# bcgsc/abyss

Hardware: AMD Instinct MI355X
Metric: Mk-mers/s inserted+extended (abyss-bloom-dbg, k=64); unitig bit-exact (higher is better)
Workload: dtype u64

## Files before the change

abyss_amd/_lib.py:

```python
from __future__ import annotations

import ctypes as C
import os

from . import build

ABG_OK = 0
ABG_EINVAL, ABG_ENODEV, ABG_ENOMEM, ABG_EINTERNAL, ABG_EAGAIN = -1, -2, -3, -4, -5


class Params(C.Structure):
    _fields_ = [
        ("k", C.c_uint32), ("num_hashes", C.c_uint32), ("min_cov", C.c_uint32), ("trim", C.c_uint32),
        ("bloom_bytes", C.c_uint64), ("counters", C.c_uint64), ("spaced_seed", C.c_char_p),
        ("device", C.c_int32), ("verbose", C.c_int32), ("insert_batch_kmers", C.c_uint64),
        ("claim_log2", C.c_uint32), ("walk_slots", C.c_uint32), ("wtab_log2", C.c_uint32),
        ("cascade_levels", C.c_uint32), ("slice_filter", C.c_uint32), ("reserved_", C.c_uint32 * 5),
    ]


class Counters(C.Structure):
    _fields_ = [(n, C.c_uint64) for n in
                ("solid_reads", "visited_reads", "reads_processed", "bases_assembled", "next_contig_id")]


class Contig(C.Structure):
    _fields_ = [
        ("contig_id", C.c_uint64), ("read_index", C.c_uint64), ("seq", C.c_char_p),
        ("length", C.c_uint32), ("coverage", C.c_uint32), ("redundant", C.c_int32),
        ("left_ext", C.c_uint32), ("right_ext", C.c_uint32), ("left_code", C.c_int32),
        ("right_code", C.c_int32), ("seed_pos", C.c_uint32),
    ]


class Stats(C.Structure):
    _fields_ = [(n, C.c_uint64) for n in
                ("insert_rounds", "walk_rounds", "candidates", "walked", "rewalked", "commit_breaks",
                 "commit_rounds", "generated", "bulk_calls", "bulk_steps", "lin_steps", "guide_slots", "chain_steps", "batch_cuts", "overflows", "memo_hits", "memo_adds", "tiled_ops", "tiled_pending", "tile_overflows", "cls_covered_reads", "archive_bases", "cls_decided_reads", "counter_bytes_held",
                 "commit_rounds_incremental", "commit_dirty_records", "commit_first_chunk_decided")]


CONTIG_CB = C.CFUNCTYPE(None, C.c_void_p, C.POINTER(Contig))
TEXT_CB = C.CFUNCTYPE(None, C.c_void_p, C.POINTER(C.c_char), C.c_uint64)

_lib = None


def symbols():
    return [
        "abg_params_init", "abg_create", "abg_destroy", "abg_last_error", "abg_reset", "abg_filter_size",
        "abg_load_seqs", "abg_load_seqs_v", "abg_keep_reads", "abg_assemble_kept", "abg_load_packed", "abg_counting_stats", "abg_counters_export",
        "abg_counters_import", "abg_visited_export", "abg_visited_import", "abg_assemble_seqs", "abg_assemble_seqs_v",
        "abg_assemble_packed", "abg_cascade_export", "abg_get_counters", "abg_set_counters", "abg_hash_seq",
        "abg_contains_seq",
        "abg_attach_comm", "abg_share_reads", "abg_rccl_unique_id", "abg_rccl_comm_create", "abg_rccl_comm_destroy",
        "abg_dev_copy", "abg_dev_alloc", "abg_dev_free", "abg_output_graph_seqs",
        "abg_profile_enable", "abg_profile_reset", "abg_profile_get", "abg_get_stats",
        "abg_overlap_create", "abg_overlap_destroy", "abg_overlap_last_error", "abg_overlap_join", "abg_overlap_edges",
        "abg_overlap_profile", "abg_overlap_profile_get",
        "abg_rr_create", "abg_rr_destroy", "abg_rr_last_error", "abg_rr_bytes", "abg_rr_clear", "abg_rr_insert_seqs",
        "abg_rr_contains_seqs", "abg_rr_popcount", "abg_rr_export", "abg_rr_sync", "abg_rr_profile", "abg_rr_profile_get",
        "abg_kn_create", "abg_kn_destroy", "abg_kn_last_error", "abg_kn_import", "abg_kn_export", "abg_kn_insert_seqs",
        "abg_kn_contains_seqs", "abg_kn_popcount", "abg_kn_hash_seq", "abg_kn_sync", "abg_kn_profile", "abg_kn_profile_get",
        "abg_fm_create", "abg_fm_destroy", "abg_fm_last_error", "abg_fm_build", "abg_fm_size", "abg_fm_export", "abg_fm_map_seqs",
        "abg_fm_sync", "abg_fm_tune", "abg_fm_profile", "abg_fm_profile_get",
        "abg_de_create", "abg_de_destroy", "abg_de_last_error", "abg_de_set_pmf", "abg_de_scan", "abg_de_estimate", "abg_de_tune",
        "abg_de_profile", "abg_de_profile_get",
        "abg_ov_create", "abg_ov_destroy", "abg_ov_last_error", "abg_ov_set_contigs", "abg_ov_find", "abg_ov_profile",
        "abg_ov_profile_get",
        "abg_sg_create", "abg_sg_destroy", "abg_sg_last_error", "abg_sg_set_graph", "abg_sg_search", "abg_sg_tune", "abg_sg_profile",
        "abg_sg_profile_get",
        "abg_mc_create", "abg_mc_destroy", "abg_mc_last_error", "abg_mc_set_contigs", "abg_mc_merge", "abg_mc_tune", "abg_mc_profile",
        "abg_mc_profile_get",
        "abg_pb_create", "abg_pb_destroy", "abg_pb_last_error", "abg_pb_tune", "abg_pb_align", "abg_pb_align_chain", "abg_pb_profile_get",
        "abg_pb_profile_reset",
    ]


def load(path: str | None = None):
    global _lib
    if _lib is not None:
        return _lib
    if path is None:
        path = os.environ.get("ABG_LIB") or build.LIB
        if not os.path.exists(path):
            build.build_lib()
    lib = C.CDLL(path)
    vp, u64p, u8p = C.c_void_p, C.POINTER(C.c_uint64), C.c_void_p
    lib.abg_params_init.argtypes = [C.POINTER(Params)]
    lib.abg_params_init.restype = None
    lib.abg_create.argtypes = [C.POINTER(Params), C.POINTER(vp)]
    lib.abg_destroy.argtypes = [vp]
    lib.abg_destroy.restype = None
    lib.abg_last_error.argtypes = [vp]
    lib.abg_last_error.restype = C.c_char_p
    lib.abg_reset.argtypes = [vp]
    lib.abg_contains_seq.argtypes = [vp, C.c_char_p, C.c_uint64, vp, vp, C.c_uint64, u64p]
    lib.abg_filter_size.argtypes = [vp, u64p]
    lib.abg_load_seqs.argtypes = [vp, C.c_char_p, vp, C.c_uint64]
    lib.abg_load_packed.argtypes = [vp, vp, vp, vp, C.c_uint64]
    lib.abg_load_seqs_v.argtypes = [vp, C.c_uint32, vp, vp, vp]
    lib.abg_keep_reads.argtypes = [vp, C.c_int, C.c_uint64]
    lib.abg_assemble_kept.argtypes = [vp, vp, CONTIG_CB, vp]
    lib.abg_counting_stats.argtypes = [vp, u64p, u64p]
    lib.abg_counters_export.argtypes = [vp, u8p]
    lib.abg_counters_import.argtypes = [vp, u8p]
    lib.abg_visited_export.argtypes = [vp, u8p]
    lib.abg_visited_import.argtypes = [vp, u8p]
    lib.abg_assemble_seqs.argtypes = [vp, C.c_char_p, vp, C.c_uint64, vp, CONTIG_CB, vp]
    lib.abg_assemble_seqs_v.argtypes = [vp, C.c_uint32, vp, vp, vp, vp, CONTIG_CB, vp]
    lib.abg_assemble_packed.argtypes = [vp, vp, vp, vp, C.c_uint64, vp, CONTIG_CB, vp]
    lib.abg_cascade_export.argtypes = [vp, C.c_uint32, u8p]
    lib.abg_get_counters.argtypes = [vp, C.POINTER(Counters)]
    lib.abg_set_counters.argtypes = [vp, C.POINTER(Counters)]
    lib.abg_hash_seq.argtypes = [vp, C.c_char_p, C.c_uint64, vp, vp, C.c_uint64, u64p]
    lib.abg_profile_enable.argtypes = [vp, C.c_int]
    lib.abg_profile_reset.argtypes = [vp]
    lib.abg_profile_get.argtypes = [vp, C.c_char_p, C.POINTER(C.c_double), u64p]
    lib.abg_get_stats.argtypes = [vp, C.POINTER(Stats)]
    lib.abg_attach_comm.argtypes = [vp, vp]
    lib.abg_share_reads.argtypes = [vp, vp, vp, vp, C.c_uint64, C.POINTER(vp), C.POINTER(vp), C.POINTER(vp), u64p]
    lib.abg_rccl_unique_id.argtypes = [vp]
# ... 109 lines not shown
```

abyss_amd/build.py:

```python
from __future__ import annotations

import os
import shutil
import subprocess
import sys

ROOT = os.path.dirname(os.path.dirname(os.path.abspath(__file__)))
CSRC = os.path.join(ROOT, "abyss_amd", "csrc")
LIB = os.path.join(ROOT, "abyss_amd", "lib", "libabyss_amd.so")
BIN_DIR = os.path.join(ROOT, "abyss_amd", "bin")
ORACLE_DIR = os.path.join(ROOT, "oracle")
HOSTCHECK = os.path.join(ROOT, "tests", "hostcheck", "libhostcheck.so")
REFERENCE = "/root/reference"


def _newer(target: str, sources) -> bool:
    if not os.path.exists(target):
        return True
    t = os.path.getmtime(target)
    return any(os.path.getmtime(s) > t for s in sources if os.path.exists(s))


def _run(cmd, cwd=None):
    r = subprocess.run(cmd, cwd=cwd, stdout=subprocess.PIPE, stderr=subprocess.STDOUT, text=True)
# ... 23 lines not shown
    "abg_fm": ["abg_fm.hip", "abg_fm.h", "abg_core.h"],
    "abg_de": ["abg_de.hip", "abg_de.h", "abg_core.h"],
    "abg_ov": ["abg_ov.hip", "abg_ov.h", "abg_core.h"],
    "abg_sg": ["abg_sg.hip", "abg_sg.h", "abg_core.h"],
    "abg_mc": ["abg_mc.hip", "abg_mc.h", "abg_ov.h", "abg_core.h"],
    "abg_pb": ["abg_pb.hip", "abg_pb.h", "abg_mc.h", "abg_ov.h", "abg_core.h"],
}
UNIT_FLAGS = {"abg_de": ["-ffp-contract=off"]}


def build_lib(force: bool = False) -> str:
    os.makedirs(OBJ_DIR, exist_ok=True)
    header = os.path.join(ROOT, "include", "abyss_amd.h")
    objs, procs = [], []
    for unit, deps in UNITS.items():
        obj = os.path.join(OBJ_DIR, unit + ".o")
        objs.append(obj)
        if force or _newer(obj, [os.path.join(CSRC, d) for d in deps] + [header]):
            cmd = [hipcc(), "--offload-arch=gfx950", "-O3", "-std=c++17", "-fPIC"] + UNIT_FLAGS.get(unit, []) + \
                ["-c", "-o", obj, os.path.join(CSRC, unit + ".hip")]
            procs.append((cmd, subprocess.Popen(cmd, stdout=subprocess.PIPE, stderr=subprocess.STDOUT, text=True)))
    for cmd, p in procs:
        out, _ = p.communicate()
        if p.returncode != 0:
            sys.stderr.write(out)
            raise RuntimeError("build step failed: %s" % " ".join(cmd))
    if force or procs or _newer(LIB, objs):
        _run([hipcc(), "--offload-arch=gfx950", "-shared", "-fPIC", "-o", LIB] + objs)
    return LIB


def build_cli(force: bool = False) -> str:
    src = os.path.join(CSRC, "host", "bloom_dbg_main.cc")
    out = os.path.join(BIN_DIR, "abyss-bloom-dbg")
    if not os.path.exists(src):
        return ""
    deps = [src] + [os.path.join(CSRC, "host", f) for f in os.listdir(os.path.join(CSRC, "host"))]
    if force or _newer(out, deps + [LIB]):
        os.makedirs(BIN_DIR, exist_ok=True)
        build_lib()
        _run(["g++", "-std=c++17", "-O2", "-I" + os.path.join(ROOT, "include"), "-o", out, src,
              "-L" + os.path.dirname(LIB), "-labyss_amd", "-Wl,-rpath,$ORIGIN/../lib", "-lpthread"])
        _run(["g++", "-std=c++17", "-O2", "-I" + os.path.join(ROOT, "include"), "-o",
              os.path.join(BIN_DIR, "abyss-bloom"), os.path.join(CSRC, "host", "bloom_main.cc"),
              "-L" + os.path.dirname(LIB), "-labyss_amd", "-Wl,-rpath,$ORIGIN/../lib", "-lpthread"])
        _run(["g++", "-std=c++17", "-O2", "-I" + os.path.join(ROOT, "include"), "-o",
              os.path.join(BIN_DIR, "AdjList"), os.path.join(CSRC, "host", "adjlist_main.cc"),
              "-L" + os.path.dirname(LIB), "-labyss_amd", "-Wl,-rpath,$ORIGIN/../lib", "-lpthread"])
        _run(["g++", "-std=c++17", "-O2", "-I" + os.path.join(ROOT, "include"), "-o",
              os.path.join(BIN_DIR, "abyss-rresolver-short"), os.path.join(CSRC, "host", "rresolver_main.cc"),
              "-L" + os.path.dirname(LIB), "-labyss_amd", "-Wl,-rpath,$ORIGIN/../lib", "-lpthread"])
        for name, main in (("abyss-map", "map_main.cc"), ("abyss-index", "index_main.cc"), ("DistanceEst", "distanceest_main.cc"),
                           ("Overlap", "overlap_main.cc"), ("SimpleGraph", "simplegraph_main.cc"), ("MergeContigs", "mergecontigs_main.cc"),
                           ("PopBubbles", "popbubbles_main.cc")):
            _run(["g++", "-std=c++17", "-O2", "-I" + os.path.join(ROOT, "include"), "-o",
                  os.path.join(BIN_DIR, name), os.path.join(CSRC, "host", main),
                  "-L" + os.path.dirname(LIB), "-labyss_amd", "-Wl,-rpath,$ORIGIN/../lib", "-lpthread"] +
                 (["-ffp-contract=off"] if name == "DistanceEst" else []))
    return out


def build_oracle(force: bool = False) -> None:
    targets = ["oracle"]
    if os.path.isdir(REFERENCE):
        targets.append("ref")
    if force:
        _run(["make", "-C", ORACLE_DIR, "clean"])
    _run(["make", "-C", ORACLE_DIR, "-j8"] + targets)


READER_CHECK = os.path.join(ROOT, "tests", "hostcheck", "reader_check")
ADJLIST_CHECK = os.path.join(ROOT, "tests", "hostcheck", "adjlist_check")
RRESOLVER_CHECK = os.path.join(ROOT, "tests", "hostcheck", "rresolver_check")
KN_CHECK = os.path.join(ROOT, "tests", "hostcheck", "kn_check")
FM_CHECK = os.path.join(ROOT, "tests", "hostcheck", "fm_check")
DE_CHECK = os.path.join(ROOT, "tests", "hostcheck", "de_check")
OV_CHECK = os.path.join(ROOT, "tests", "hostcheck", "ov_check")
SG_CHECK = os.path.join(ROOT, "tests", "hostcheck", "sg_check")
MC_CHECK = os.path.join(ROOT, "tests", "hostcheck", "mc_check")
PB_CHECK = os.path.join(ROOT, "tests", "hostcheck", "pb_check")


def build_hostcheck(force: bool = False) -> str:
    src = os.path.join(ROOT, "tests", "hostcheck", "hostcheck_ext.cc")
    if force or _newer(HOSTCHECK, [src, os.path.join(ROOT, "tests", "hostcheck", "hostcheck.cc")] + csrc_files()):
        _run(["g++", "-std=c++17", "-O2", "-g", "-fPIC", "-shared", "-Wno-unknown-pragmas", "-o", HOSTCHECK, src])
    rsrc = os.path.join(ROOT, "tests", "hostcheck", "reader_check.cc")
    if force or _newer(READER_CHECK, [rsrc, os.path.join(CSRC, "host", "fasta_reader.h")]):
        _run(["g++", "-std=c++17", "-O2", "-o", READER_CHECK, rsrc])
    asrc = os.path.join(ROOT, "tests", "hostcheck", "adjlist_check.cc")
    if force or _newer(ADJLIST_CHECK, [asrc, HOSTCHECK, os.path.join(CSRC, "host", "adjlist_core.h"),
                                       os.path.join(CSRC, "host", "fasta_reader.h")]):
        _run(["g++", "-std=c++17", "-O2", "-o", ADJLIST_CHECK, asrc, "-L" + os.path.dirname(HOSTCHECK), "-lhostcheck",
              "-Wl,-rpath,$ORIGIN"])
    hsrc = [os.path.join(CSRC, "host", f) for f in ("rresolver_core.h", "graph_writers.h", "fasta_reader.h", "si_bytes.h")]
    csrc = os.path.join(ROOT, "tests", "hostcheck", "rresolver_check.cc")
    if force or _newer(RRESOLVER_CHECK, [csrc, os.path.join(CSRC, "abg_rr.h"), os.path.join(CSRC, "abg_core.h")] + hsrc):
        _run(["g++", "-std=c++17", "-O2", "-Wno-unknown-pragmas", "-o", RRESOLVER_CHECK, csrc, "-lpthread"])
    ksrc = os.path.join(ROOT, "tests", "hostcheck", "kn_check.cc")
    kdeps = [ksrc] + [os.path.join(CSRC, f) for f in ("abg_kn.h", "abg_core.h")] + \
        [os.path.join(CSRC, "host", f) for f in ("bloom_core.h", "fasta_reader.h")]
    if force or _newer(KN_CHECK, kdeps):
        _run(["g++", "-std=c++17", "-O2", "-Wno-unknown-pragmas", "-o", KN_CHECK, ksrc, "-lpthread"])
    fsrc = os.path.join(ROOT, "tests", "hostcheck", "fm_check.cc")
    fdeps = [fsrc] + [os.path.join(CSRC, f) for f in ("abg_fm.h", "abg_core.h")] + \
        [os.path.join(CSRC, "host", f) for f in ("map_core.h", "fasta_reader.h")]
    if force or _newer(FM_CHECK, fdeps):
        _run(["g++", "-std=c++17", "-O2", "-Wno-unknown-pragmas", "-o", FM_CHECK, fsrc, "-lpthread"])
    dsrc = os.path.join(ROOT, "tests", "hostcheck", "de_check.cc")
    ddeps = [dsrc] + [os.path.join(CSRC, f) for f in ("abg_de.h", "abg_core.h")] + [os.path.join(CSRC, "host", "distanceest_core.h")]
    if force or _newer(DE_CHECK, ddeps):
        _run(["g++", "-std=c++17", "-O2", "-ffp-contract=off", "-Wno-unknown-pragmas", "-o", DE_CHECK, dsrc, "-lpthread"])
    osrc = os.path.join(ROOT, "tests", "hostcheck", "ov_check.cc")
    odeps = [osrc] + [os.path.join(CSRC, f) for f in ("abg_ov.h", "abg_core.h")] + \
        [os.path.join(CSRC, "host", f) for f in ("overlap_core.h", "rresolver_core.h", "graph_writers.h", "fasta_reader.h", "si_bytes.h")]
    if force or _newer(OV_CHECK, odeps):
        _run(["g++", "-std=c++17", "-O2", "-Wno-unknown-pragmas", "-o", OV_CHECK, osrc, "-lpthread"])
    ssrc = os.path.join(ROOT, "tests", "hostcheck", "sg_check.cc")
    sdeps = [ssrc] + [os.path.join(CSRC, f) for f in ("abg_sg.h", "abg_core.h")] + \
        [os.path.join(CSRC, "host", f) for f in ("simplegraph_core.h", "overlap_core.h", "rresolver_core.h", "graph_writers.h", "fasta_reader.h", "si_bytes.h")]
    if force or _newer(SG_CHECK, sdeps):
        _run(["g++", "-std=c++17", "-O2", "-Wno-unknown-pragmas", "-o", SG_CHECK, ssrc, "-lpthread"])
    msrc = os.path.join(ROOT, "tests", "hostcheck", "mc_check.cc")
    mdeps = [msrc] + [os.path.join(CSRC, f) for f in ("abg_mc.h", "abg_ov.h", "abg_core.h")] + \
        [os.path.join(CSRC, "host", f) for f in ("mergecontigs_core.h", "overlap_core.h", "rresolver_core.h", "graph_writers.h", "fasta_reader.h", "si_bytes.h")]
    if force or _newer(MC_CHECK, mdeps):
        _run(["g++", "-std=c++17", "-O2", "-Wno-unknown-pragmas", "-o", MC_CHECK, msrc, "-lpthread"])
    psrc = os.path.join(ROOT, "tests", "hostcheck", "pb_check.cc")
    pdeps = [psrc] + [os.path.join(CSRC, f) for f in ("abg_pb.h", "abg_mc.h", "abg_ov.h", "abg_core.h")] + \
        [os.path.join(CSRC, "host", f) for f in ("popbubbles_core.h", "rresolver_core.h", "graph_writers.h", "fasta_reader.h", "si_bytes.h")]
    if force or _newer(PB_CHECK, pdeps):
        _run(["g++", "-std=c++17", "-O2", "-Wno-unknown-pragmas", "-o", PB_CHECK, psrc, "-lpthread"])
    return HOSTCHECK


def build_all(force: bool = False) -> None:
    build_lib(force)
    build_cli(force)
    build_oracle(force)
    build_hostcheck(force)


if __name__ == "__main__":
    build_all("--force" in sys.argv)
    print("built:", LIB)
```

abyss_amd/csrc/abg_core.h:

```cpp
#pragma once

#include <stdint.h>
#include <stddef.h>

#if defined(__HIPCC__)
#include <hip/hip_runtime.h>
#define ABG_HD __host__ __device__ __forceinline__
#define ABG_HDN __host__ __device__
#define ABG_HDX __host__ __device__ __attribute__((noinline))
#else
#define ABG_HD inline
#define ABG_HDN
#define ABG_HDX
#endif

namespace abg {

constexpr int MAX_NW = 6;
constexpr int MAX_HASHES = 32;
constexpr unsigned FP_TRIM = 5;

enum Dir : int { FORWARD = 0, REVERSE = 1 };
enum Sense : int { SENSE = 0, ANTISENSE = 1 };

// ... 1035 lines not shown
}

#if defined(__HIP_DEVICE_COMPILE__)
ABG_HD uint64_t ld_coherent(const uint64_t* p)
{
	return __hip_atomic_load(p, __ATOMIC_RELAXED, __HIP_MEMORY_SCOPE_AGENT);
}
ABG_HD uint32_t ld_coherent(const uint32_t* p)
{
	return __hip_atomic_load(p, __ATOMIC_RELAXED, __HIP_MEMORY_SCOPE_AGENT);
}
ABG_HD void st_coherent(uint64_t* p, uint64_t v)
{
	__hip_atomic_store(p, v, __ATOMIC_RELAXED, __HIP_MEMORY_SCOPE_AGENT);
}
ABG_HD uint64_t cas_u64(uint64_t* p, uint64_t expect, uint64_t val)
{
	return (uint64_t)atomicCAS((unsigned long long*)p, (unsigned long long)expect,
	    (unsigned long long)val);
}
ABG_HD uint32_t cas_u32(uint32_t* p, uint32_t expect, uint32_t val) { return atomicCAS(p, expect, val); }
ABG_HD uint32_t atomic_min_u32(uint32_t* p, uint32_t v) { return atomicMin(p, v); }
ABG_HD uint64_t atomic_min_u64(uint64_t* p, uint64_t v)
{
	return (uint64_t)atomicMin((unsigned long long*)p, (unsigned long long)v);
}
ABG_HD uint32_t atomic_add_u32(uint32_t* p, uint32_t v) { return atomicAdd(p, v); }
ABG_HD uint64_t atomic_add_u64(uint64_t* p, uint64_t v)
{
	return (uint64_t)atomicAdd((unsigned long long*)p, (unsigned long long)v);
}
ABG_HD uint32_t atomic_or_u32(uint32_t* p, uint32_t v) { return atomicOr(p, v); }
ABG_HD uint64_t atomic_exch_u64(uint64_t* p, uint64_t v)
{
	return (uint64_t)atomicExch((unsigned long long*)p, (unsigned long long)v);
}
#else
ABG_HD uint64_t ld_coherent(const uint64_t* p) { return *p; }
ABG_HD uint32_t ld_coherent(const uint32_t* p) { return *p; }
ABG_HD void st_coherent(uint64_t* p, uint64_t v) { *p = v; }
ABG_HD uint64_t cas_u64(uint64_t* p, uint64_t expect, uint64_t val)
{
	uint64_t old = *p;
	if (old == expect) *p = val;
	return old;
}
ABG_HD uint32_t cas_u32(uint32_t* p, uint32_t expect, uint32_t val) { uint32_t o = *p; if (o == expect) *p = val; return o; }
ABG_HD uint32_t atomic_min_u32(uint32_t* p, uint32_t v) { uint32_t o = *p; if (v < o) *p = v; return o; }
ABG_HD uint64_t atomic_min_u64(uint64_t* p, uint64_t v) { uint64_t o = *p; if (v < o) *p = v; return o; }
ABG_HD uint32_t atomic_add_u32(uint32_t* p, uint32_t v) { uint32_t o = *p; *p = o + v; return o; }
ABG_HD uint64_t atomic_add_u64(uint64_t* p, uint64_t v) { uint64_t o = *p; *p = o + v; return o; }
ABG_HD uint32_t atomic_or_u32(uint32_t* p, uint32_t v) { uint32_t o = *p; *p = o | v; return o; }
ABG_HD uint64_t atomic_exch_u64(uint64_t* p, uint64_t v) { uint64_t o = *p; *p = v; return o; }
#endif

#if defined(__HIP_DEVICE_COMPILE__)
ABG_HD uint32_t wave_append_slot(uint32_t* counter, bool want)
{
	const uint64_t m = __ballot(want ? 1 : 0);
	if (m == 0) return 0;
	const unsigned lane = __lane_id();
	const int leader = __ffsll((unsigned long long)m) - 1;
	uint32_t base = 0;
	if ((int)lane == leader) base = atomicAdd(counter, (uint32_t)__popcll(m));
	base = (uint32_t)__shfl((int)base, leader);
	return base + (uint32_t)__popcll(m & ((1ull << lane) - 1));
}
#else
ABG_HD uint32_t wave_append_slot(uint32_t* counter, bool want)
{
	if (!want) return 0;
	uint32_t o = *counter; *counter = o + 1; return o;
}
#endif

#if defined(__HIP_DEVICE_COMPILE__)
ABG_HD void wave_count_add(uint64_t* counter, bool want)
{
	const uint64_t m = __ballot(want ? 1 : 0);
	if (m && (int)__lane_id() == __ffsll((unsigned long long)m) - 1) atomicAdd((unsigned long long*)counter, (unsigned long long)__popcll(m));
}
#else
ABG_HD void wave_count_add(uint64_t* counter, bool want) { if (want) *counter += 1; }
#endif

#if defined(__HIP_DEVICE_COMPILE__)
ABG_HD uint32_t wave_rank(bool want, uint32_t& count)
{
	const uint64_t m = __ballot(want ? 1 : 0);
	count = (uint32_t)__popcll(m);
	return (uint32_t)__popcll(m & ((1ull << __lane_id()) - 1));
}
#else
ABG_HD uint32_t wave_rank(bool want, uint32_t& count) { count = want ? 1u : 0u; return 0; }
#endif

#if defined(__HIP_DEVICE_COMPILE__)
ABG_HD void wave_put_bit(uint64_t* words, uint32_t i, bool v)
{
	const uint64_t m = __ballot(v ? 1 : 0);
	if (!(i & 63u)) words[i >> 6] = m;
}
#else
ABG_HD void wave_put_bit(uint64_t* words, uint32_t i, bool v)
{
	if (!(i & 63u)) words[i >> 6] = 0;
	words[i >> 6] |= (uint64_t)(v ? 1u : 0u) << (i & 63u);
}
#endif

#if defined(__HIP_DEVICE_COMPILE__)
ABG_HD uint64_t wu_cas_u64(uint64_t* p, uint64_t expect, uint64_t val, bool coop)
{
	if (!coop) return cas_u64(p, expect, val);
	uint64_t r = 0;
	if (__lane_id() == 0) r = cas_u64(p, expect, val);
	return ((uint64_t)(uint32_t)__builtin_amdgcn_readfirstlane((int)(r >> 32)) << 32) |
	       (uint32_t)__builtin_amdgcn_readfirstlane((int)(uint32_t)r);
}
ABG_HD uint32_t wu_atomic_min_u32(uint32_t* p, uint32_t v, bool coop)
{
	if (!coop) return atomic_min_u32(p, v);
	uint32_t r = 0;
	if (__lane_id() == 0) r = atomic_min_u32(p, v);
	return (uint32_t)__builtin_amdgcn_readfirstlane((int)r);
}
ABG_HD uint32_t wu_atomic_add_u32(uint32_t* p, uint32_t v, bool coop)
{
	if (!coop) return atomic_add_u32(p, v);
	uint32_t r = 0;
	if (__lane_id() == 0) r = atomic_add_u32(p, v);
	return (uint32_t)__builtin_amdgcn_readfirstlane((int)r);
}
ABG_HD uint64_t wu_atomic_add_u64(uint64_t* p, uint64_t v, bool coop)
{
	if (!coop) return atomic_add_u64(p, v);
	uint64_t r = 0;
	if (__lane_id() == 0) r = atomic_add_u64(p, v);
	return ((uint64_t)(uint32_t)__builtin_amdgcn_readfirstlane((int)(r >> 32)) << 32) |
	       (uint32_t)__builtin_amdgcn_readfirstlane((int)(uint32_t)r);
}
ABG_HD void wu_st_coherent(uint64_t* p, uint64_t v, bool coop)
{
	if (!coop || __lane_id() == 0) st_coherent(p, v);
}
ABG_HD void wu_st_u32(uint32_t* p, uint32_t v, bool coop)
{
	if (!coop || __lane_id() == 0) *p = v;
}
ABG_HD void wu_st_u8(uint8_t* p, uint8_t v, bool coop)
{
	if (!coop || __lane_id() == 0) *p = v;
}
#else
ABG_HD void wu_st_coherent(uint64_t* p, uint64_t v, bool) { st_coherent(p, v); }
ABG_HD void wu_st_u32(uint32_t* p, uint32_t v, bool) { *p = v; }
ABG_HD void wu_st_u8(uint8_t* p, uint8_t v, bool) { *p = v; }
ABG_HD uint64_t wu_cas_u64(uint64_t* p, uint64_t e, uint64_t v, bool) { return cas_u64(p, e, v); }
ABG_HD uint32_t wu_atomic_min_u32(uint32_t* p, uint32_t v, bool) { return atomic_min_u32(p, v); }
ABG_HD uint32_t wu_atomic_add_u32(uint32_t* p, uint32_t v, bool) { return atomic_add_u32(p, v); }
ABG_HD uint64_t wu_atomic_add_u64(uint64_t* p, uint64_t v, bool) { return atomic_add_u64(p, v); }
#endif

struct Guide {
	const uint64_t* tab;
	uint64_t mask;
// ... 966 lines not shown
```

abyss_amd/csrc/abg_engine.h:

```cpp
#pragma once
#include "abg_walk.h"

#include <algorithm>
#include <chrono>
#include <cstdio>
#include <cstdlib>
#include <cstring>
#include <functional>
#include <future>
#include <string>
#include <type_traits>
#include <vector>

namespace abg {

struct Failure { int code; std::string msg; };
constexpr int FAIL_INVAL = -1, FAIL_NOMEM = -3, FAIL_INTERNAL = -4;
[[noreturn]] inline void fail_now(int code, const std::string& msg) { throw Failure{ code, msg }; }
inline std::string strf(const char* fmt, unsigned long long a = 0, unsigned long long b = 0)
{
	char buf[256];
	snprintf(buf, sizeof buf, fmt, a, b);
	return buf;
}

struct Config {
	uint32_t k = 0, nh = 4, kc = 2, trim = 0;
	uint64_t counters = 0;
	uint32_t cascade_levels = 0;
	std::string spaced_seed;
	uint64_t insert_batch_kmers = 1ull << 24;
	uint32_t claim_log2 = 30;
	uint32_t drain_threshold = 1u << 12;
	uint64_t compact_threshold = 1u << 20;
	bool async_load = true;
	bool tiled_insert = true;
	bool benign_sharers = true;
	uint32_t cls_debug_skip = 0;
	bool cls_archive = true;
	uint32_t cls_archive_max_mb = 16384;
	bool sorted_overflow = true;
	bool cosettle = true;
	uint32_t cosettle_passes = 6;
	uint32_t cosettle_log2 = 24;
	uint32_t walk_slots = 4096;
	uint32_t tb_cap = 512;
	uint32_t buf_cap = 1u << 16;
	uint64_t pool_cap = 1ull << 28;
	uint32_t rec_cap = 1u << 22;
	uint32_t wtab_log2 = 26;
	uint32_t wtab_log2_max = 31;
	uint32_t cend_log2 = 20;
	uint64_t p2_first_batch = 65536;
	uint64_t p2_max_batch = 1ull << 22;
	uint32_t p2_growth = 2;
	uint32_t p2_crowded = 1u << 18;
	uint32_t p2_starved_growth = 2;
	uint32_t p2_starved = 6144;
	uint32_t slice_filter = 0;
	bool solid_plane = true;
	uint32_t classify_slots = 65536;
	uint32_t cls_both_max_mb = 1024;
	bool cls_both = true;
	bool prefetch_classify = true;
	uint32_t memo_log2 = 0;
	bool memo = true;
	uint32_t p2_max_candidates = 1u << 18;
	uint32_t t_tags = 1024;
	uint32_t commit_incremental = 1;
	uint32_t commit_dirty_max = 4096;
	uint32_t commit_dirty_log2 = 26;
	uint32_t guide_stride = 4;
	uint32_t guide_log2_max = 31;
	bool guide_seen = true;
	bool link_duplicates = true;
	bool par_commit = true;
	bool overlap_bins = true;
	bool overlap_purity = true;
	bool apply_mask = true;
	bool lead_implicit = true;
	uint32_t dist_hash_all_ranks = 2;
	uint32_t dist_route_min_ranks = 4;
	uint64_t keep_insert_scratch_bytes = 16ull << 30;
	uint64_t par_commit_max_bytes = 16ull << 30;
	int verbose = 0;
};

struct Counters {
	uint64_t solid_reads = 0, visited_reads = 0, reads_processed = 0, bases_assembled = 0,
	         contig_id = 0;
};

struct BaseCodes {
	uint8_t t[256];
	BaseCodes()
	{
		for (int i = 0; i < 256; i++) t[i] = 0xFF;
		t['A'] = t['a'] = 0; t['C'] = t['c'] = 1; t['G'] = t['g'] = 2; t['T'] = t['t'] = 3;
	}
};
template <class T>
struct NoInitAlloc : std::allocator<T> {
	template <class U> struct rebind { using other = NoInitAlloc<U>; };
	template <class U, class... A> void construct(U* p, A&&... a)
	{
		if constexpr (sizeof...(A) == 0) ::new ((void*)p) U; else ::new ((void*)p) U(std::forward<A>(a)...);
	}
};
struct HostBatch {
	std::vector<uint32_t, NoInitAlloc<uint32_t>> words;
	std::vector<uint64_t> woff{ 0 };
	std::vector<uint32_t> len;
	std::vector<uint64_t> koff{ 0 };
	void clear() { words.clear(); woff.assign(1, 0); len.clear(); koff.assign(1, 0); }
	uint64_t n() const { return len.size(); }
	void add_ascii(const char* s, uint32_t L, uint32_t k)
	{
		static const BaseCodes codes;
		uint64_t w0 = words.size();
		words.resize(w0 + (L + 15) / 16);
		uint32_t* out = words.data() + w0;
		uint32_t i = 0;
		for (; i + 16 <= L; i += 16) {
			uint32_t w = 0;
			for (uint32_t j = 0; j < 16; j++) w |= (uint32_t)(codes.t[(unsigned char)s[i + j]] & 3u) << (2 * j);
			*out++ = w;
		}
		if (i < L) {
			uint32_t w = 0;
			for (uint32_t j = 0; i + j < L; j++) w |= (uint32_t)(codes.t[(unsigned char)s[i + j]] & 3u) << (2 * j);
			*out = w;
		}
		woff.push_back(words.size());
		len.push_back(L);
		koff.push_back(koff.back() + (L - k + 1));
	}
};

struct ContigOut {
	uint64_t contig_id;
	uint64_t read_index;
	std::string seq;
	uint32_t coverage;
	bool redundant;
	uint32_t left_ext, right_ext;
	int left_code, right_code;
	uint32_t seed_pos;
};

ABG_HD uint64_t claim_val(uint32_t epoch, uint32_t t) { return ((uint64_t)(0xFFFFFFFFu - epoch) << 32) | t; }

struct FHash {
	Params p; Batch b; uint64_t* h0;
	ABG_HD void operator()(uint64_t t, uint32_t) const
	{
		uint64_t r = find_seq(b.koff, b.n, t);
		uint32_t j = (uint32_t)(t - b.koff[r]);
		h0[t] = scratch_hash(p, [&](unsigned i) { return batch_base(b, r, j + i); });
// ... 1533 lines not shown
	{
		const uint32_t L = b.len[r];
		if (L < p.k) return;
		const uint32_t nk = L - p.k + 1;
		const uint64_t woff = b.woff[r];
		if (nk > GUIDE_MAX_NK || woff > GUIDE_MAX_WOFF) return;
		if (!p.mask) {
			constexpr uint32_t RUN = 8;
			for (uint32_t j0 = lane * RUN; j0 < nk; j0 += nlanes * RUN) {
				const uint32_t j1 = j0 + RUN < nk ? j0 + RUN : nk;
				uint64_t hm[RUN];
				for (uint32_t q = 0; q < RUN; q++) hm[q] = 0;
				kmer_hash_run(p, [&](unsigned q) { return batch_base(b, r, q); }, j0, j1, [&](uint32_t j, uint64_t h) { hm[j - j0] = h; });
				unsigned c[RUN];
#pragma unroll
				for (uint32_t q = 0; q < RUN; q++) c[q] = probe_c(p, cnt, pos_i(p, hm[j0 + q < j1 ? q : 0u], 0));
#pragma unroll
				for (uint32_t q = 0; q < RUN; q++)
					if (j0 + q < j1 && c[q] >= p.kc) tab[guide_slot(hm[q], mask)] = guide_pack(woff, j0 + q, nk, guide_tag(hm[q]));
			}
			return;
		}
		for (uint32_t j = lane; j < nk; j += nlanes) {
			const Kmer<NW> s = window_kmer<NW>(b.words, woff, j, p.k);
			uint64_t fh, rh;
			kmer_hashes(s, p.k, fh, rh);
			const uint64_t hm = rh < fh ? rh : fh;
			uint64_t df = 0, dr = 0;
			if constexpr (MASKED_BUILD<NW>) masked_terms(p, s, df, dr);
			const uint64_t fs = fh ^ df, rs = rh ^ dr;
			if (probe_c(p, cnt, pos_i(p, rs < fs ? rs : fs, 0)) < p.kc) continue;
			tab[guide_slot(hm, mask)] = guide_pack(woff, j, nk, guide_tag(hm));
		}
	}
};

constexpr uint32_t WALK_FAST_WITH_CACHE = 16384;
template <int NW>
struct FWalk {
	WalkEnv<NW> e; const uint32_t* list;
	ABG_HDN void operator()(uint64_t i, uint32_t slot, void* fast, uint32_t fast_bytes, bool coop)
	{
		WalkEnv<NW>* env = (WalkEnv<NW>*)fast;
		const uint32_t a = (uint32_t)((sizeof(WalkEnv<NW>) + 15) & ~15ull);
		*env = e;
		env->mcache = nullptr;
		if (fast_bytes >= WALK_FAST_WITH_CACHE) {
			fast_bytes -= (uint32_t)sizeof(MaskCache);
			env->mcache = (MaskCache*)((char*)fast + fast_bytes);
		}
		env->fast = (char*)fast + a;
		env->fast_bytes = fast_bytes - a;
		env->coop = coop;
		walk_read<NW>(*env, list[i], slot);
	}
};

template <int NW>
ABG_HDN uint64_t seq_kmer_hash(const Params& p, const uint8_t* seq, uint64_t j)
{
	return scratch_hash(p, [&](unsigned i) { return (unsigned)seq[j + i]; });
}
template <int NW>
ABG_HDN uint64_t read_kmer_hash(const Params& p, const Batch& b, uint64_t r, uint32_t j)
{
	return scratch_hash(p, [&](unsigned i) { return batch_base(b, r, j + i); });
}
constexpr uint32_t PREP_RUN = 8;
ABG_HD uint64_t dup_mix(uint64_t x) { x ^= x >> 31; x *= 0xD6E8FEB86659FD93ULL; x ^= x >> 29; x *= 0x9E3779B97F4A7C15ULL; x ^= x >> 32; return x | 1; }
template <int NW>
struct FReadPrep {
	Params p; Batch b; const uint32_t* cand_read; const uint64_t* rkoff; uint64_t* rkh; uint32_t first;
	ABG_HDN void operator()(uint64_t i, uint32_t lane, uint32_t nlanes) const
	{
		uint32_t c = first + (uint32_t)i;
		uint64_t r = cand_read[c];
		uint32_t nk = b.len[r] - p.k + 1;
		uint64_t* out = rkh + rkoff[c];
		for (uint32_t j0 = lane * PREP_RUN; j0 < nk; j0 += nlanes * PREP_RUN)
			kmer_hash_run(p, [&](unsigned q) { return batch_base(b, r, q); }, j0, j0 + PREP_RUN < nk ? j0 + PREP_RUN : nk,
			    [&](uint32_t j, uint64_t h) { out[j] = h; });
	}
};
template <int NW>
struct FContigPrep {
	Params p; const uint8_t* cnt; ContigRec* recs; uint32_t first; const uint8_t* pool; uint64_t* kh;
	uint32_t with_cov;
	ABG_HDN void operator()(uint64_t i, uint32_t lane, uint32_t nlanes) const
	{
		ContigRec& rec = recs[first + i];
		const uint8_t* seq = pool + rec.seq_off;
		uint64_t* out = kh + rec.seq_off;
		uint32_t cnk = rec.len - p.k + 1;
		uint32_t cov = 0;
		uint64_t fp = 0;
		for (uint32_t j0 = lane * PREP_RUN; j0 < cnk; j0 += nlanes * PREP_RUN)
			kmer_hash_run(p, [&](unsigned q) { return (unsigned)seq[q]; }, j0, j0 + PREP_RUN < cnk ? j0 + PREP_RUN : cnk,
			    [&](uint32_t j, uint64_t h) { out[j] = h; fp += dup_mix(h); if (with_cov) cov += solid_min_count(p, cnt, h); });
		if (cov) atomic_add_u32(&rec.coverage, cov);
		if (fp) atomic_add_u64(&rec.fp, fp);
	}
};

struct FDupKeys {
	const ContigRec* recs; uint32_t k; uint64_t* key; uint32_t* val;
	ABG_HD void operator()(uint64_t i, uint32_t) const
	{
		const ContigRec& r = recs[i];
		key[i] = r.len < k + FP_TRIM - 1 ? ~0ULL - i : dup_mix(r.fp ^ ((uint64_t)r.len << 40));
		val[i] = (uint32_t)i;
	}
};
struct FDupLink {
	ContigRec* recs; const uint64_t* key; const uint32_t* val; uint64_t n; uint32_t first_new;
	ABG_HD void operator()(uint64_t q, uint32_t) const
	{
		const uint32_t me = val[q];
		if (me < first_new) return;
		const uint64_t k = key[q];
		uint64_t g = q;
		for (unsigned s = 0; s < 64 && g > 0 && key[g - 1] == k; s++) g--;
		uint32_t best = REC_END, best_cand = recs[me].cand;
		for (unsigned s = 0; s < 128 && g < n && key[g] == k; s++, g++) {
			const uint32_t o = val[g];
			if (o != me && recs[o].cand < best_cand && recs[o].len == recs[me].len && recs[o].fp == recs[me].fp) { best = o; best_cand = recs[o].cand; }
		}
		recs[me].dup_of = best;
	}
};
struct FDupVerify {
	ContigRec* recs; const uint64_t* kh; uint32_t k; uint32_t first_new;
	ABG_HDN void operator()(uint64_t i, uint32_t lane, uint32_t nlanes) const
	{
		ContigRec& d = recs[first_new + i];
		const uint32_t o = d.dup_of;
		if (o == REC_END) return;
		const uint64_t* a = kh + d.seq_off; const uint64_t* b = kh + recs[o].seq_off;
		const uint32_t nk = d.len - k + 1;
		bool fwd = true, rev = true;
		for (uint32_t j = lane; j < nk; j += nlanes) { const uint64_t x = a[j]; fwd = fwd & (x == b[j]); rev = rev & (x == b[nk - 1 - j]); }
		fwd = wave_all_lanes(fwd, nlanes); rev = wave_all_lanes(rev, nlanes);
		if (!fwd && !rev && lane == 0) d.dup_of = REC_END;
	}
};
constexpr uint32_t PC_SCAN_RUN = 4;
template <class Test>
ABG_HD bool wave_all_kmers(uint32_t n, uint32_t lane, uint32_t nlanes, Test test, bool& first_chunk)
{
	bool mine = lane < n ? test(lane) : true;
	first_chunk = !wave_all_lanes(mine, nlanes);
	if (first_chunk) return false;
	for (uint32_t j0 = nlanes; j0 < n; j0 += PC_SCAN_RUN * nlanes) {
#pragma unroll
		for (uint32_t u = 0; u < PC_SCAN_RUN; u++) {
			const uint32_t j = j0 + u * nlanes + lane;
			if (j < n) mine = mine & test(j);
		}
		if (!wave_all_lanes(mine, nlanes)) return false;
	}
	return true;
}
ABG_HD bool visited_contains_owned(const Params& p, const uint8_t* __restrict__ vis, uint64_t h, uint64_t lo, uint64_t span)
{
	bool ok = true;
	if (p.nh <= 4) {
		uint64_t q4[4]; uint8_t b4[4];
#pragma unroll
		for (unsigned i = 0; i < 4; i++) { q4[i] = pos_i(p, h, i < p.nh ? i : 0u); b4[i] = vis[q4[i] >> 3]; }
#pragma unroll
		for (unsigned i = 0; i < 4; i++) if (i < p.nh && q4[i] - lo < span) ok = ok & (((b4[i] >> (q4[i] & 7)) & 1u) != 0);
		return ok;
	}
	for (unsigned i = 0; i < p.nh; i++) {
		const uint64_t q = pos_i(p, h, i);
		if (q - lo < span) ok = ok & (((vis[q >> 3] >> (q & 7)) & 1u) != 0);
	}
	return ok;
}
template <int NW>
struct FPreCommit {
	Params p; Batch b; const uint32_t* cand_read; const uint32_t* status; const uint32_t* first_rec;
	ContigRec* recs; const uint8_t* vis; const uint64_t* kh; const uint64_t* rkh; const uint64_t* rkoff;
	uint8_t* read_flag; uint32_t first;
	uint64_t lo, span; uint8_t* part_c; uint8_t* part_r;
	uint32_t* nfirst;
	ABG_HDN void operator()(uint64_t i, uint32_t lane, uint32_t nlanes) const
	{
		uint32_t c = first + (uint32_t)i;
		uint64_t r = cand_read[c];
		uint32_t nk = b.len[r] - p.k + 1;
		const uint64_t* rh = rkh + rkoff[c];
		bool fc;
		const bool all = wave_all_kmers(nk, lane, nlanes, [&](uint32_t j) { return visited_contains_owned(p, vis, rh[j], lo, span); }, fc);
		uint32_t nf = fc ? 1u : 0u;
		if (nfirst && lane == 0) nfirst[i] = nf;
		if (part_c) {
			if (lane == 0) part_c[i] = all ? 1 : 0;
			if (status[c] != WS_COMPLETE) return;
		} else {
			if (lane == 0) read_flag[c] = all ? 1 : 0;
			if (all || status[c] != WS_COMPLETE) return;
		}
		for (uint32_t ri = first_rec[c]; ri != REC_END; ri = recs[ri].next) {
			ContigRec& rec = recs[ri];
			uint32_t cnk = rec.len - p.k + 1;
			if (rec.len < p.k + FP_TRIM - 1 || rec.pre_redundant) continue;
			if (rec.dup_of != REC_END && recs[rec.dup_of].cand >= first) continue;
			const uint64_t* ch = kh + rec.seq_off;
			const bool red = wave_all_kmers(cnk, lane, nlanes, [&](uint32_t j) { return visited_contains_owned(p, vis, ch[j], lo, span); }, fc);
			nf += fc ? 1u : 0u;
			if (part_r) { if (lane == 0) part_r[ri] = red ? 1 : 0; }
			else if (lane == 0 && red) rec.pre_redundant = 1;
		}
		if (nfirst && lane == 0) nfirst[i] = nf;
	}
};
struct FPreCommitCopies {
	const uint32_t* status; const uint32_t* first_rec; ContigRec* recs; const uint8_t* read_flag; uint32_t first; uint32_t k;
	ABG_HD void operator()(uint64_t i, uint32_t) const
	{
		const uint32_t c = first + (uint32_t)i;
		if (read_flag[c] || status[c] != WS_COMPLETE) return;
		for (uint32_t ri = first_rec[c]; ri != REC_END; ri = recs[ri].next) {
			ContigRec& rec = recs[ri];
			if (rec.len < k + FP_TRIM - 1 || rec.pre_redundant || rec.dup_of == REC_END) continue;
// ... 847 lines not shown
				kmin[rec.seq_off + j] = (uint8_t)mn;
			}
			if (sum && cov) atomic_add_u32(&rec.coverage, cov);
		}
	}
};
struct FPcWrite {
	ParCommit e; uint32_t* order; uint32_t order_base; uint64_t id_base;
	ABG_HD void operator()(uint64_t i, uint32_t) const
	{
		const uint32_t c = e.c_begin + (uint32_t)i;
		if (c >= e.brk || !e.active[i]) return;
		uint32_t o = order_base + e.cnt[i];
		uint64_t id = id_base + e.cnt2[i];
		for (uint32_t ri = e.first_rec[c]; ri != REC_END; ri = e.recs[ri].next) {
			ContigRec& rec = e.recs[ri];
			order[o++] = ri;
			if (rec.ins) rec.contig_id = id++;
		}
	}
};

template <class BE>
class Engine {
  public:
	Engine(BE& be, const Config& cfg) : be_(be), cfg_(cfg)
	{
		uint64_t rem = cfg_.counters % 8;
		m_ = rem ? cfg_.counters + 8 - rem : cfg_.counters;
		p_ = make_params(cfg_.k, cfg_.nh, cfg_.kc, cfg_.trim, m_);
		if (!cfg_.spaced_seed.empty()) {
			MaskTab* mt = new MaskTab;
			make_mask(cfg_.spaced_seed.c_str(), cfg_.k, *mt, p_);
			mask_d_ = (MaskTab*)be_.alloc(sizeof(MaskTab));
			be_.h2d(mask_d_, mt, sizeof(MaskTab));
			delete mt;
			p_.mask = mask_d_;
		}
		if (cfg_.cascade_levels) {
			casc_.levels = cfg_.cascade_levels;
			casc_.level_words = (m_ + 31) / 32;
			casc_.bits = (uint32_t*)be_.alloc(casc_.levels * casc_.level_words * 4);
			be_.memset(casc_.bits, 0, casc_.levels * casc_.level_words * 4);
			cnt_ = (uint8_t*)be_.alloc(8);
			vis_bytes_ = 8;
		} else {
			const uint64_t dev = be_.device_mem_bytes();
			cnt_deferred_ = cfg_.slice_filter == 1 || (cfg_.slice_filter == 0 && dev && (double)m_ * 1.3 > (double)dev * 0.9);
			if (!cnt_deferred_) {
				cnt_ = (uint8_t*)be_.alloc(m_ + 64 * (MAX_RANKS + 1));
				be_.memset(cnt_, 0, m_);
			}
			vis_bytes_ = (m_ / 8 + 4 + 3) & ~3ull;
		}
		vis_ = (uint8_t*)be_.alloc(vis_bytes_);
		be_.memset(vis_, 0, vis_bytes_);
		cstate_ = (CommitState*)be_.alloc(sizeof(CommitState));
		be_.memset(cstate_, 0, sizeof(CommitState));
		scal_ = (uint64_t*)be_.alloc(64);
	}
	~Engine()
	{
		if (BE::ITEM_GROUP_LOG2 == 0 && getenv("ABG_LEAD_COUNT"))
			fprintf(stderr, "lead_stores made=%llu skipped=%llu\n", (unsigned long long)stats_.lead_stores[0], (unsigned long long)stats_.lead_stores[1]);
		free_counters(); be_.free(vis_); if (both_) be_.free(both_); be_.free(cstate_); be_.free(scal_);
		free_archive();
		if (casc_.bits) be_.free(casc_.bits);
		if (mask_d_) be_.free(mask_d_);
		if (T_) be_.free(T_);
		if (Tk_) { be_.free(Tk_); be_.free(Tv_); }
		if (pcA_) be_.free(pcA_);
		if (la_pool_c_) be_.free(la_pool_c_);
		if (la_pool_c2_) be_.free(la_pool_c2_);
		if (guide_tab_) be_.free(guide_tab_);
		if (guide_seen_) be_.free(guide_seen_);
		if (gtab_.hmin) free_tab(gtab_);
		free_shared();
		free_insert();
		free_walk();
		if (cend_.hmin) free_tab(cend_);
		if (memo_tab_.hmin) free_tab(memo_tab_);
		if (plane_) be_.free(plane_);
		if (wstats_) be_.free(wstats_);
	}
	void reset()
	{
		if (casc_.bits) be_.memset(casc_.bits, 0, casc_.levels * casc_.level_words * 4);
		else if (sliced_) be_.memset(cnt_ + own_lo_, 0, own_span_);
		else if (cnt_) be_.memset(cnt_, 0, m_);
		be_.memset(vis_, 0, vis_bytes_);
		arc_valid_ = false; loaded_ops_ = 0;
		be_.memset(cstate_, 0, sizeof(CommitState));
		counters_ = Counters();
		stats_ = Stats();
		cnt_partial_ = false; cnt_loaded_ = false;
		memo_valid_ = false; plane_valid_ = false;
		last_rounds_ = 0;
		p2_batch_ = cfg_.p2_first_batch;
		last_candidates_ = 0;
		if (cend_.hmin) {
			be_.memset(cend_.hmin, 0xFF, (cend_.mask + 1) * 8);
			be_.memset(cend_.meta, 0xFF, (cend_.mask + 1) * 8);
		}
		cend_count_ = 0;
		if (wstats_) clear_wstats();
		ovf_seen_[0] = ovf_seen_[1] = 0;
		if (gtab_.hmin) { free_tab(gtab_); gtab_ = WalkTab{ nullptr, nullptr, nullptr, 0 }; gtab_used_ = 0; }
	}
	const Params& params() const { return p_; }
	uint64_t size() const { return m_; }
	uint8_t* counters_dev() { need_whole_filter("direct access to the counters"); gather_counters(); memo_valid_ = false; plane_valid_ = false; arc_valid_ = false;  return cnt_; }

	struct Comm {
		int rank = 0, world = 1;
		bool stream_ordered = false;
		void* user = nullptr;
		int (*all_gather_v)(void*, void*, const uint64_t*, const uint64_t*, void*) = nullptr;
		int (*all_reduce)(void*, void*, uint64_t, int32_t, int32_t, void*) = nullptr;
		int (*all_to_all_v)(void*, const void*, const uint64_t*, const uint64_t*, void*, const uint64_t*, const uint64_t*, void*) = nullptr;
	};
	enum { DT_U8 = 0, DT_U32 = 1, DT_U64 = 2, OP_SUM = 0, OP_MAX = 1, OP_MIN = 2 };
	bool attach_comm(const Comm& c)
	{
		if (c.world < 1 || c.world > MAX_RANKS || c.rank < 0 || c.rank >= c.world || casc_.bits) return false;
		uint64_t chunk = (m_ + c.world - 1) / c.world;
		chunk = (chunk + 63) & ~63ull;
		if (sliced_ && cnt_loaded_ && (c.rank != comm_.rank || c.world != comm_.world))
			fail_now(FAIL_INVAL, "a sliced filter that holds counters cannot take a communicator with another rank or world (abg_counters_export / _import move them)");
		const bool keep_window = sliced_ && c.rank == comm_.rank && c.world == comm_.world && own_chunk_ == chunk;
		comm_ = c;
		free_insert();
		own_lo_ = std::min<uint64_t>(m_, (uint64_t)c.rank * chunk);
		own_span_ = std::min<uint64_t>(m_, own_lo_ + chunk) - own_lo_;
		own_chunk_ = chunk;
		if (sliced_ || cnt_deferred_) {
			if (!cfg_.solid_plane || (m_ & 63) || !cfg_.par_commit)
				fail_now(FAIL_INVAL, "a sliced filter needs the bit plane, the parallel commit and a multiple of 64 counters");
			if (!keep_window) {
				free_counters();
				if (plane_) { be_.free(plane_); plane_ = nullptr; }
				win_total_ = (uint64_t)c.world * chunk + 64;
				win_span_ = chunk + 64;
				win_lo_ = own_lo_;
				cnt_ = (uint8_t*)be_.alloc_window(win_total_, win_lo_, win_span_);
				be_.memset(cnt_ + own_lo_, 0, win_span_);
				cnt_loaded_ = false;
			}
			sliced_ = true; cnt_deferred_ = false;
			cfg_.drain_threshold = 0;
			memo_valid_ = false; plane_valid_ = false;
		}
		const char* f = getenv("ABG_FORCE_DIST");
		force_dist_ = f && atoi(f) != 0;
		if (c.world > 1 && !comm_scaled_) {
			comm_scaled_ = true;
			cfg_.p2_first_batch *= (uint64_t)c.world;
			cfg_.p2_max_batch *= (uint64_t)c.world;
			cfg_.p2_starved *= (uint32_t)c.world;
			cfg_.p2_crowded *= (uint32_t)std::min(c.world, 4);
			p2_batch_ = cfg_.p2_first_batch;
		}
		return true;
	}
	bool dist() const { return comm_.world > 1 || force_dist_ || sliced_; }
	bool sliced() const { return sliced_; }
	uint64_t counter_bytes_held() const { return sliced_ ? win_span_ : cnt_ ? m_ : 0; }
	void need_counters() const
	{
		if (!cnt_) fail_now(FAIL_INVAL, "this filter does not fit the device: attach a communicator first, its ranks keep a range each (abg_attach_comm)");
	}
	void need_whole_filter(const char* what) const
	{
		need_counters();
		if (sliced_) fail_now(FAIL_INVAL, std::string(what) + " is not available on a sliced filter (each rank holds a range of the counters)");
	}
	void free_counters()
	{
		if (sliced_) be_.free_window(cnt_, win_total_, win_lo_, win_span_);
		else if (cnt_) be_.free(cnt_);
		cnt_ = nullptr; sliced_ = false;
	}
	Batch share_reads(const Batch& loc)
	{
		const uint32_t R = (uint32_t)comm_.world, me = (uint32_t)comm_.rank;
		uint64_t w0 = 0, w1 = 0;
		if (loc.n) { be_.d2h(&w0, loc.woff, 8); be_.d2h(&w1, loc.woff + loc.n, 8); }
		std::vector<uint64_t> cnt(2 * R, 0);
		cnt[2 * me] = loc.n; cnt[2 * me + 1] = w1 - w0;
// ... 322 lines not shown
	{
		const bool want = cfg_.cls_archive && !dist() && !sliced_ && !casc_.bits && b.n && use_par_commit();
		if (!want) { free_archive(); return; }
		const uint64_t nk = loaded_ops_ ? loaded_ops_ : m_ / 4;
		uint64_t cap = std::max<uint64_t>(nk / 4, 1ull << 16) + ARC_HEAD, slots = 1ull << 12;
		while (slots < cap / 2) slots <<= 1;
		const uint64_t budget = (uint64_t)cfg_.cls_archive_max_mb << 20;
		while (slots > (1ull << 12) && slots * 8 + cap > budget) { slots >>= 1; cap = std::min(cap, slots * 2); }
		if (cap >= (1ULL << ARC_POS_BITS)) cap = (1ULL << ARC_POS_BITS) - 1;
		if (arc_.seq && (arc_.cap < cap || arc_.mask + 1 < slots)) free_archive();
		if (!arc_.seq) {
			arc_.seq = (uint8_t*)be_.try_alloc(cap + ARC_PAD);
			arc_.tab = (uint64_t*)be_.try_alloc(slots * 8);
			arc_.used = (uint64_t*)be_.try_alloc(8);
			if (!arc_.seq || !arc_.tab || !arc_.used) {
				if (arc_.seq) be_.free(arc_.seq); if (arc_.tab) be_.free(arc_.tab); if (arc_.used) be_.free(arc_.used);
				arc_ = ContigArchive();
				return;
			}
			arc_.cap = cap; arc_.mask = slots - 1;
			arc_valid_ = false;
		}
		arc_.nreads = wstats_ ? wstats_ + WSTAT_CLS_COVERED : nullptr;
		if (!arc_valid_) {
			be_.memset(arc_.seq, ARC_SEP, arc_.cap + ARC_PAD);
			be_.memset(arc_.tab, 0, (arc_.mask + 1) * 8);
			const uint64_t head = ARC_HEAD;
			be_.h2d(arc_.used, &head, 8);
			arc_valid_ = true;
		}
	}
	ContigArchive arc_{}; bool arc_valid_ = false;
	uint64_t loaded_ops_ = 0;
	uint64_t ovf_seen_[2] = { 0, 0 };
	uint8_t* plane_ = nullptr; bool plane_valid_ = false;
	Params p2_; const uint8_t* cnt2_ = nullptr;

	void build_guide(const Batch& b)
	{
		guide_.tab = nullptr; guide_.seen = nullptr; guide_slots_ = 0;
		if (!cfg_.guide_stride || p_.nh > 8 || !b.n) return;
		const uint64_t sampled = (b.n + cfg_.guide_stride - 1) / cfg_.guide_stride;
		uint64_t nwords = 0;
		be_.d2h(&nwords, b.woff + b.n, 8);
		const uint64_t bases = nwords * 16, minus = b.n * (uint64_t)(p_.k - 1);
		const uint64_t kmers = (bases > minus ? bases - minus : b.n) / std::min<uint32_t>(cfg_.guide_stride, 4u);
		uint32_t log2 = 16;
		while ((1ull << log2) < kmers && log2 < cfg_.guide_log2_max) log2++;
		if (!guide_tab_ || log2 != guide_log2_) {
			if (guide_tab_) be_.free(guide_tab_);
			guide_tab_ = (uint64_t*)be_.try_alloc(8ull << log2);
			guide_log2_ = log2;
			if (!guide_tab_) { if (cfg_.verbose) fprintf(stderr, "abyss_amd: no memory for the walkers' guide table, walking step by step\n"); return; }
		}
		be_.memset(guide_tab_, 0, 8ull << log2);
		guide_.mask = (1ull << log2) - 1; guide_.words = b.words; guide_.nwords = nwords;
		dispatch_nw([&](auto nw) {
			FGuideBuild<decltype(nw)::value> f{ p2_, b, cnt2_, guide_tab_, guide_.mask, cfg_.guide_stride, sampled };
			be_.launch_wave((sampled + GUIDE_READS_PER_ITEM - 1) / GUIDE_READS_PER_ITEM, f, "guide_build");
		});
		guide_.tab = guide_tab_;
		guide_slots_ = guide_.mask + 1;
		if (cfg_.guide_seen) {
			const uint64_t need = nwords * 16, total = be_.device_mem_bytes();
			if (guide_seen_ && guide_seen_bytes_ < need) { be_.free(guide_seen_); guide_seen_ = nullptr; }
			if (!guide_seen_ && (!total || need <= total / 24)) { guide_seen_ = (uint8_t*)be_.try_alloc(need); guide_seen_bytes_ = need; }
			if (guide_seen_) { be_.memset(guide_seen_, 0, need); guide_.seen = guide_seen_; }
		}
	}
	uint64_t next_batch_size() const
	{
		if (last_candidates_ > cfg_.p2_crowded) return std::max<uint64_t>(p2_batch_ / 2, 1024);
		if (last_candidates_ < cfg_.p2_starved) return std::min<uint64_t>(p2_batch_ * cfg_.p2_starved_growth, 8 * cfg_.p2_max_batch);
		return std::min<uint64_t>(p2_batch_ * cfg_.p2_growth, cfg_.p2_max_batch);
	}
	void clear_wstats()
	{
		be_.memset(wstats_, 0, WSTAT_N * 8);
	}
	struct Stats { uint64_t rounds = 0, walked = 0, rewalked = 0, candidates = 0, breaks = 0, insert_rounds = 0, commit_rounds = 0, generated = 0;
	               uint64_t bulk_calls = 0, bulk_steps = 0, lin_steps = 0, guide_slots = 0, chain_steps = 0, batch_cuts = 0, overflows = 0, memo_hits = 0, memo_adds = 0;
	               uint64_t tiled_ops = 0, tiled_pending = 0, tile_overflows = 0, cls_covered_reads = 0, archive_bases = 0, cls_decided_reads = 0;
	               uint64_t lead_stores[2] = { 0, 0 };
	               uint64_t commit_rounds_incremental = 0, commit_dirty_records = 0, commit_first_chunk_decided = 0; };
	Stats stats()
	{
		Stats s = stats_;
		if (wstats_) {
			uint64_t v[WSTAT_N];
			be_.d2h(v, wstats_, sizeof v);
			s.bulk_calls = v[WSTAT_BULK_CALLS]; s.bulk_steps = v[WSTAT_BULK_STEPS]; s.lin_steps = v[WSTAT_LIN_STEPS]; s.chain_steps = v[WSTAT_CHAIN_STEPS];
			s.memo_hits = v[WSTAT_MEMO_HITS]; s.memo_adds = v[WSTAT_MEMO_ADDS];
			s.cls_covered_reads = v[WSTAT_CLS_COVERED]; s.cls_decided_reads = v[WSTAT_CLS_DECIDED];
		}
		if (arc_.seq && arc_valid_) { uint64_t u = 0; be_.d2h(&u, arc_.used, 8); s.archive_bases = std::min(u, arc_.cap) - ARC_HEAD; }
		s.guide_slots = guide_slots_;
		return s;
	}

  private:
	BE& be_;
	Config cfg_;
	Params p_;
	uint64_t m_ = 0, vis_bytes_ = 0;
	uint8_t* cnt_ = nullptr;
	uint8_t* vis_ = nullptr;
	CommitState* cstate_ = nullptr;
	uint64_t* scal_ = nullptr;
	Cascade casc_{ nullptr, 0, 0 };
	MaskTab* mask_d_ = nullptr;
	std::chrono::steady_clock::time_point dbg_t0_;
	uint32_t* T_ = nullptr;
	uint32_t t_tag_ = 0;
	uint64_t* Tk_ = nullptr; uint32_t* Tv_ = nullptr; uint32_t Tlog2_ = 0;
	uint64_t T_entries_ = 0;
	uint32_t* pcA_ = nullptr; uint64_t pcA_bits_ = 0; uint32_t pcA_shift_ = 0;
	bool t_hashed() const { return t_force_hashed_ || m_ * 4ull > cfg_.par_commit_max_bytes; }
	bool t_force_hashed_ = false;
	bool use_par_commit()
	{
		if (!cfg_.par_commit || t_failed_) return false;
		if (t_hashed()) return true;
		if (!T_) {
			T_ = (uint32_t*)be_.try_alloc(m_ * 4ull);
			t_tag_ = 0;
			if (!T_ && sliced_) {
				t_force_hashed_ = true;
				if (cfg_.verbose) fprintf(stderr, "abyss_amd: no memory for a time stamp per filter bit, hashed stamps instead\n");
				return true;
			}
			if (!T_) { t_failed_ = true; if (cfg_.verbose) fprintf(stderr, "abyss_amd: no memory for the parallel commit's time stamps, using the ordered kernel\n"); return false; }
		}
		return true;
	}
	bool t_failed_ = false;
	Comm comm_;
	bool force_dist_ = false, comm_scaled_ = false;
	bool sliced_ = false, cnt_deferred_ = false; uint64_t win_total_ = 0, win_span_ = 0, win_lo_ = 0;
	bool cnt_loaded_ = false;
	uint64_t own_lo_ = 0, own_span_ = 0, own_chunk_ = 0;
	uint8_t* tred_ = nullptr;
	bool cnt_partial_ = false;
	uint32_t* sh_words_ = nullptr; uint64_t* sh_woff_ = nullptr; uint32_t* sh_len_ = nullptr; uint64_t* sh_koff_ = nullptr;
	uint8_t* dres_ = nullptr; uint8_t* dlost_ = nullptr;
	TilePair* rsend_ = nullptr; TilePair* rrecv_ = nullptr; uint32_t rcap_ = 0; uint64_t rrecv_cap_ = 0; uint32_t* rslot_ = nullptr; uint32_t* rcur_ = nullptr;
	uint8_t* rrep_out_ = nullptr; uint8_t* rrep_in_ = nullptr; uint8_t* rtgt_out_ = nullptr; uint8_t* rtgt_in_ = nullptr; uint8_t* rpendf_ = nullptr;
	uint64_t rown_ = 0;
	bool routed() const
	{
		return dist() && cfg_.dist_route_min_ranks && (uint32_t)comm_.world >= cfg_.dist_route_min_ranks && (comm_.all_to_all_v || comm_.world == 1) && p_.nh <= 16;
	}
	uint32_t g_rec_ = 0; uint64_t g_pool_ = 0;
  public:
  private:
	void free_shared()
	{
		if (!sh_words_) return;
		be_.free(sh_words_); be_.free(sh_woff_); be_.free(sh_len_); be_.free(sh_koff_);
		sh_words_ = nullptr;
	}
	void c_fail(const char* what) { fail_now(FAIL_INTERNAL, std::string("collective ") + what + " failed on rank " + std::to_string(comm_.rank)); }
	void c_all_gather_v(void* buf, const uint64_t* counts, const uint64_t* displs)
	{
		if (!comm_.stream_ordered) be_.sync();
		be_.begin("comm_all_gather");
		if (comm_.all_gather_v(comm_.user, buf, counts, displs, be_.stream_handle())) c_fail("all_gather_v");
		be_.end("comm_all_gather");
	}
	void c_all_reduce(void* buf, uint64_t n, int dtype, int op)
	{
		if (!n) return;
		if (!comm_.stream_ordered) be_.sync();
		be_.begin("comm_all_reduce");
		if (comm_.all_reduce(comm_.user, buf, n, dtype, op, be_.stream_handle())) c_fail("all_reduce");
		be_.end("comm_all_reduce");
	}
	void c_all_to_all_v(const void* send, const uint64_t* sc, const uint64_t* sd, void* recv, const uint64_t* rc, const uint64_t* rd)
	{
		if (comm_.world == 1) {
			if (sc[0]) be_.d2d((char*)recv + rd[0], (const char*)send + sd[0], sc[0]);
			return;
		}
		if (!comm_.stream_ordered) be_.sync();
		be_.begin("comm_all_to_all");
		if (comm_.all_to_all_v(comm_.user, send, sc, sd, recv, rc, rd, be_.stream_handle())) c_fail("all_to_all_v");
		be_.end("comm_all_to_all");
	}
	void host_all_reduce_sum(uint64_t* v, uint32_t n)
	{
		uint64_t* d = (uint64_t*)be_.alloc(n * 8ull);
		be_.h2d(d, v, n * 8ull);
		c_all_reduce(d, n, DT_U64, OP_SUM);
		be_.d2h(v, d, n * 8ull);
		be_.free(d);
	}
	void gather_counters()
	{
		if (!dist() || !cnt_partial_ || sliced_) return;
		std::vector<uint64_t> c(comm_.world), d(comm_.world);
		for (int q = 0; q < comm_.world; q++) { d[q] = (uint64_t)q * own_chunk_; c[q] = own_chunk_; }
		c_all_gather_v(cnt_, c.data(), d.data());
		cnt_partial_ = false;
	}
	Counters counters_;
	Stats stats_;
	uint64_t last_rounds_ = 0;
	uint64_t p2_batch_ = 0;
	uint64_t* h0_ = nullptr; uint64_t* claim_[2] = { nullptr, nullptr };
	uint32_t* pend_[2] = { nullptr, nullptr }; uint32_t* pend_n_ = nullptr; uint32_t epoch_ = 1;
	uint64_t batch_ops_ = 0;
	uint32_t hash_run_ = 8;
	uint64_t insert_scratch_bytes_ = 0;
	uint32_t claim_log2_ = 0;
	bool tiled_ = false; uint64_t ntiles_ = 0, napply_ = 0; uint32_t tile_cap_ = 0;
	TilePair* coarse_ = nullptr; uint32_t* ccur_ = nullptr; uint32_t coarse_cap_ = 0, cshift_ = 0, ncoarse_ = 0;
	TilePair* bins_ = nullptr; uint32_t* tcur_ = nullptr; uint32_t* lead_ = nullptr; uint8_t* opflag_ = nullptr; uint8_t* tgt_ = nullptr; uint8_t* pendf_ = nullptr;
	uint64_t* h0_alt_ = nullptr; TilePair* bins_alt_ = nullptr; uint32_t* tcur_alt_ = nullptr;
	uint32_t* colist_ = nullptr; uint8_t* cocnt_ = nullptr;
	uint64_t* pgrp_ = nullptr;
	uint8_t* wmask_ = nullptr; uint32_t* bad_ = nullptr; uint32_t* cochg_ = nullptr;
	uint32_t* lead_alt_ = nullptr; uint8_t* opflag_alt_ = nullptr;
	uint64_t* amask_ = nullptr; uint64_t* amask_alt_ = nullptr;
	bool staged_purity_ = false;
	Guide guide_{ nullptr, 0, nullptr, 0, nullptr }; uint64_t* guide_tab_ = nullptr; uint32_t guide_log2_ = 0;
	uint8_t* guide_seen_ = nullptr; uint64_t guide_seen_bytes_ = 0;
	BulkScratch* bulk_pool_ = nullptr; uint64_t* wstats_ = nullptr; uint64_t guide_slots_ = 0;
	SuccMemo memo_{ nullptr, nullptr, nullptr, 0 }; WalkTab memo_tab_{ nullptr, nullptr, nullptr, 0 }; bool memo_valid_ = false; uint64_t memo_gen_ = 0;
	bool walk_ready_ = false;
	WalkTab wtab_{}, cend_{ nullptr, nullptr, nullptr, 0 };
	uint32_t wtab_log2_ = 0;
	uint64_t wtab_per_walker_ = 1536;
	void* tb_pool_ = nullptr; VKey* tbk_pool_ = nullptr; VKey* la_pool_ = nullptr; uint8_t* lbuf_ = nullptr; uint8_t* rbuf_ = nullptr;
	uint8_t* pool_ = nullptr; uint64_t pool_cap_ = 0; uint64_t* pool_used_ = nullptr;
	ContigRec* recs_ = nullptr; uint32_t rec_cap_ = 0; uint32_t* rec_used_ = nullptr;
	uint32_t* order_ = nullptr; uint32_t* order_n_ = nullptr;
	uint32_t walk_tb_cap_ = 0, walk_buf_cap_ = 0, wslots_ = 0, cslots_ = 0;
	uint64_t* kh_ = nullptr; uint64_t* rkh_ = nullptr; uint64_t* dbg_ = nullptr;
	uint64_t cend_count_ = 0;
	uint8_t* read_flag_ = nullptr;
	uint64_t last_candidates_ = 0;
	VKey* la_pool_c_ = nullptr;
	VKey* la_pool_c2_ = nullptr;
	uint64_t pre_first_ = 0, pre_n_ = 0;
	std::function<void()> prefetch_;

	WalkTab gtab_{ nullptr, nullptr, nullptr, 0 };
	uint64_t gtab_used_ = 0;
	template <class F>
	void dispatch_nw(F&& f)
	{
		switch (p_.mask ? NW_MASKED + p_.nw : p_.nw) {
		case 1: f(std::integral_constant<int, 1>()); break;
		case 2: f(std::integral_constant<int, 2>()); break;
		case 3: f(std::integral_constant<int, 3>()); break;
		case 4: f(std::integral_constant<int, 4>()); break;
		case 5: case 6: f(std::integral_constant<int, 6>()); break;
		case NW_MASKED + 1: f(std::integral_constant<int, NW_MASKED + 1>()); break;
		case NW_MASKED + 2: f(std::integral_constant<int, NW_MASKED + 2>()); break;
		case NW_MASKED + 3: f(std::integral_constant<int, NW_MASKED + 3>()); break;
		case NW_MASKED + 4: f(std::integral_constant<int, NW_MASKED + 4>()); break;
		default: f(std::integral_constant<int, NW_MASKED + 6>()); break;
		}
	}
	template <int NW>
	void graph_bfs_nw(const Batch& starts, const Batch& marks, std::vector<uint8_t>& ev, std::vector<uint8_t>& used, uint64_t* edges)
	{
		if (!gtab_.hmin) { alloc_tab(gtab_, 16); gtab_used_ = 0; }
		uint64_t node_cap = 1ull << 16;
		GNode<NW>* nodes = (GNode<NW>*)be_.alloc(node_cap * sizeof(GNode<NW>));
		uint8_t* ev_d = (uint8_t*)be_.alloc(node_cap);
		uint8_t* used_d = (uint8_t*)be_.alloc(starts.n);
		GraphState* st_d = (GraphState*)be_.alloc(sizeof(GraphState));
		GraphState st;
		memset(&st, 0, sizeof st);
		st.tab_used = gtab_used_;
		be_.h2d(st_d, &st, sizeof st);
		for (;;) {
			FGraphBfs<NW> f{ p_, cnt_, starts, marks, starts.n, gtab_, (gtab_.mask + 1) / 2, nodes, node_cap, ev_d, used_d, st_d };
			be_.launch(1, f, "graph_bfs");
			be_.d2h(&st, st_d, sizeof st);
			if (st.stop == 1) {
				nodes = (GNode<NW>*)regrow(nodes, node_cap * sizeof(GNode<NW>), 2 * node_cap * sizeof(GNode<NW>));
				ev_d = (uint8_t*)regrow(ev_d, node_cap, 2 * node_cap);
				node_cap *= 2;
			} else if (st.stop == 2) {
				uint32_t log2 = 1;
				while ((1ull << log2) < gtab_.mask + 1) log2++;
				WalkTab bigger{};
				alloc_tab(bigger, log2 + 1);
				uint32_t* failed = (uint32_t*)be_.alloc(8);
				be_.memset(failed, 0, 4);
				FRehash fr{ gtab_, bigger, failed };
				be_.launch(gtab_.mask + 1, fr, "rehash");
				uint32_t bad = 0;
				be_.d2h(&bad, failed, 4);
				be_.free(failed);
				if (bad) fail_now(FAIL_INTERNAL, "graph table rehash failed");
				free_tab(gtab_);
				gtab_ = bigger;
			} else {
				break;
			}
		}
		gtab_used_ = st.tab_used;
		ev.resize(st.count);
		be_.d2h(ev.data(), ev_d, st.count);
		be_.d2h(used.data(), used_d, starts.n);
		*edges = st.edges;
		be_.free(nodes); be_.free(ev_d); be_.free(used_d); be_.free(st_d);
// ... 450 lines not shown
		if (nown) be_.compact_flagged(nullptr, rpendf_, nown, pend_[0], pend_n_);
		uint32_t mine = 0;
		be_.d2h(&mine, pend_n_, 4);
		std::vector<uint64_t> pc(R, 0);
		pc[me] = mine;
		host_all_reduce_sum(pc.data(), (uint32_t)R);
		uint64_t npend = 0;
		std::vector<uint64_t> gc(R), gd(R);
		for (uint64_t q = 0; q < R; q++) { gd[q] = npend * sizeof(TilePair); gc[q] = pc[q] * sizeof(TilePair); npend += pc[q]; }
		stats_.tiled_ops += T; stats_.tiled_pending += npend;
		if (npend) {
			TilePair* g = rsend_;
			TilePair* big = nullptr;
			if (npend > R * (uint64_t)rcap_) { big = (TilePair*)be_.alloc(npend * sizeof(TilePair)); g = big; }
			if (mine) { FRoutePendRec f{ h0_, pend_[0], a, (TilePair*)((char*)g + gd[me]) }; be_.launch(mine, f, "route_pend"); }
			c_all_gather_v(g, gc.data(), gd.data());
			FRoutePendTake f{ g, h0_, pend_[1] };
			be_.launch(npend, f, "route_pend");
			if (big) { be_.sync(); be_.free(big); }
			FClaimOwned fc{ p_, h0_, pend_[1], claim_[0], cmask, epoch_, own_lo_, own_span_ };
			be_.launch(npend, fc, "claim_list");
		}
		insert_rounds_dist(T, cmask, pend_[1], npend);
	}
	void insert_rounds_dist(uint64_t T, uint64_t cmask, const uint32_t* pin, uint64_t npend)
	{
		(void)T;
		cnt_partial_ = true;
		uint64_t* ccur = claim_[0];
		uint64_t* cnext = claim_[1];
		uint32_t* pout = pend_[0];
		while (npend) {
			if (pin && npend <= cfg_.drain_threshold) {
				uint8_t* val = dres_;
				{ FDrainVals f{ p_, h0_, cnt_, pin, own_lo_, own_span_, val }; be_.launch(npend, f, "drain_vals"); }
				c_all_reduce(val, npend * p_.nh, DT_U8, OP_MAX);
				{ FDrainLoad f{ p_, h0_, cnt_, pin, own_lo_, own_span_, val, ccur, cmask, epoch_ }; be_.launch(npend, f, "drain_load"); }
				uint32_t* other = (pin == pend_[0]) ? pend_[1] : pend_[0];
				InsertDrainEnv de{ p_, h0_, cnt_, casc_, const_cast<uint32_t*>(pin), other, (uint32_t)npend,
					ccur, cnext, cmask, epoch_, pend_n_ };
				be_.launch_drain(de);
				uint32_t r[2] = { 0, 0 };
				be_.d2h(r, pend_n_, 8);
				epoch_ += r[1];
				last_rounds_ += r[1];
				stats_.insert_rounds += r[1];
				break;
			}
			{ FEvalDist f{ p_, h0_, cnt_, pin, ccur, cmask, epoch_, own_lo_, own_span_, dres_ }; be_.launch(npend, f, pin ? "insert_retry" : "insert_round"); }
			c_all_reduce(dres_, npend, DT_U8, OP_MIN);
			{ FApplyDist f{ p_, h0_, cnt_, pin, cnext, cmask, epoch_, own_lo_, own_span_, dres_, dlost_ }; be_.launch(npend, f, "insert_apply"); }
			be_.compact_flagged(pin, dlost_, npend, pout, pend_n_);
			uint32_t nn = 0;
			be_.d2h(&nn, pend_n_, 4);
			npend = nn;
			std::swap(ccur, cnext);
			pin = pout;
			pout = (pout == pend_[0]) ? pend_[1] : pend_[0];
			epoch_++;
			last_rounds_++;
			stats_.insert_rounds++;
		}
		epoch_++;
	}

	void ensure_walk()
	{
		if (walk_ready_) return;
		if (!cend_.hmin) {
			p2_batch_ = cfg_.p2_first_batch;
			cslots_ = std::min<uint32_t>(be_.max_slots(), cfg_.classify_slots);
			alloc_tab(cend_, cfg_.cend_log2);
		}
		wslots_ = std::min<uint32_t>(be_.max_slots(), cfg_.walk_slots);
		wtab_log2_ = cfg_.wtab_log2;
		alloc_tab(wtab_, wtab_log2_);
		la_pool_ = (VKey*)be_.alloc((uint64_t)wslots_ * LA_MAX_VISITED * sizeof(VKey));
		bulk_pool_ = (BulkScratch*)be_.alloc((uint64_t)wslots_ * sizeof(BulkScratch));
		if (!wstats_) { wstats_ = (uint64_t*)be_.alloc(WSTAT_N * 8); clear_wstats(); }
		walk_tb_cap_ = cfg_.tb_cap;
		walk_buf_cap_ = cfg_.buf_cap;
		alloc_walk_scratch();
		pool_cap_ = cfg_.pool_cap;
		pool_ = (uint8_t*)be_.alloc(pool_cap_);
		kh_ = (uint64_t*)be_.alloc(pool_cap_ * 8);
		pool_used_ = (uint64_t*)be_.alloc(8);
		rec_cap_ = cfg_.rec_cap;
		recs_ = (ContigRec*)be_.alloc((uint64_t)rec_cap_ * sizeof(ContigRec));
		rec_used_ = (uint32_t*)be_.alloc(8);
		order_ = (uint32_t*)be_.alloc((uint64_t)rec_cap_ * 4);
		order_n_ = (uint32_t*)be_.alloc(8);
		walk_ready_ = true;
	}
	void alloc_walk_scratch()
	{
		tb_pool_ = be_.alloc((uint64_t)wslots_ * walk_tb_cap_ * sizeof(TBFrame<NW_MASKED + MAX_NW>));
		tbk_pool_ = (VKey*)be_.alloc((uint64_t)wslots_ * walk_tb_cap_ * sizeof(VKey));
		lbuf_ = (uint8_t*)be_.alloc((uint64_t)wslots_ * walk_buf_cap_);
		rbuf_ = (uint8_t*)be_.alloc((uint64_t)wslots_ * walk_buf_cap_);
	}
	void free_walk_scratch() { be_.free(tb_pool_); be_.free(tbk_pool_); be_.free(lbuf_); be_.free(rbuf_); }
	void alloc_tab(WalkTab& t, uint32_t log2)
	{
		uint64_t cap = 1ull << log2;
		t.hmin = (uint64_t*)be_.alloc(cap * 8);
		t.hmax = (uint64_t*)be_.alloc(cap * 8);
		t.meta = (uint64_t*)be_.alloc(cap * 8);
		t.mask = cap - 1;
		be_.memset(t.hmin, 0xFF, cap * 8);
		be_.memset(t.meta, 0xFF, cap * 8);
	}
	void free_tab(WalkTab& t) { be_.free(t.hmin); be_.free(t.hmax); be_.free(t.meta); }
	void free_walk()
	{
		if (!walk_ready_) return;
		free_tab(wtab_);
		be_.free(la_pool_); be_.free(bulk_pool_);
		free_walk_scratch();
		be_.free(pool_); be_.free(kh_); be_.free(pool_used_); be_.free(recs_); be_.free(rec_used_);
		be_.free(order_); be_.free(order_n_);
		walk_ready_ = false;
	}
	void grow_walk_resources()
	{
		free_walk_scratch();
		walk_tb_cap_ *= 4;
		walk_buf_cap_ *= 8;
		if (walk_buf_cap_ > (1u << 28) || wtab_log2_ > 31) {
			fail_now(FAIL_INTERNAL, "a unitig exceeds the walker limits");
		}
		while ((uint64_t)wslots_ * walk_buf_cap_ > (8ull << 30) && wslots_ > 64) wslots_ /= 2;
		alloc_walk_scratch();
		free_tab(wtab_);
		wtab_log2_++;
		alloc_tab(wtab_, wtab_log2_);
		be_.free(pool_); be_.free(kh_);
		pool_cap_ *= 2;
		pool_ = (uint8_t*)be_.alloc(pool_cap_);
		kh_ = (uint64_t*)be_.alloc(pool_cap_ * 8);
		if (cfg_.verbose)
			fprintf(stderr, "abyss_amd: walker resources grown: %u frames, %u bases, 2^%u table, %llu pool\n",
			    walk_tb_cap_, walk_buf_cap_, wtab_log2_, (unsigned long long)pool_cap_);
	}

	template <int NW>
	WalkEnv<NW> make_env(const Batch& b, uint32_t* cand_d, uint32_t* status_d, uint32_t* first_d)
	{
		WalkEnv<NW> e;
		e.p = p2_; e.cnt = cnt2_; e.batch = b; e.cand_read = cand_d; e.status = status_d; e.first_rec = first_d;
		e.tab = wtab_; e.owner_base = 0;
		e.tb_pool = (TBFrame<NW>*)tb_pool_;
		e.tbk_pool = tbk_pool_;
		e.tb_cap = walk_tb_cap_;
		e.fast = nullptr; e.fast_bytes = 0; e.dbg = dbg_; e.coop = false;
		e.la_pool = la_pool_;
		e.guide = guide_; e.bulk_pool = bulk_pool_; e.wstats = wstats_; e.memo = memo_; e.mcache = nullptr;
		e.lbuf_pool = lbuf_; e.rbuf_pool = rbuf_; e.buf_cap = walk_buf_cap_;
		e.pool = pool_; e.pool_cap = pool_cap_; e.pool_used = pool_used_;
		e.recs = recs_; e.rec_cap = rec_cap_; e.rec_used = rec_used_;
		return e;
	}

	template <int NW>
	uint32_t commit(const Batch& b, uint32_t* cand_d, uint32_t* status_d, uint32_t* first_d,
	    uint8_t* result_d, const uint64_t* rkoff_d, uint32_t c_begin, uint32_t c_end)
	{
		{
			uint32_t nrec = 0, nord = 0;
			be_.d2h(&nrec, rec_used_, 4);
			be_.d2h(&nord, order_n_, 4);
			uint64_t need = cend_count_ + 2ull * (std::min(nrec, rec_cap_) - std::min(nord, rec_cap_));
			while (need * 2 > cend_.mask + 1) grow_cend();
		}
		CommitState cs;
		cs.counters = counters_;
		cs.break_at = c_begin; cs.pad_ = 0; cs.cend_count = cend_count_;
		be_.h2d(cstate_, &cs, sizeof cs);
		{
			FPreCommit<NW> f{ p_, b, cand_d, status_d, first_d, recs_, vis_, kh_, rkh_, rkoff_d, read_flag_, c_begin, 0, ~0ULL, nullptr, nullptr, nullptr };
			be_.launch_wave(c_end - c_begin, f, "precommit");
			FPreCommitCopies fc{ status_d, first_d, recs_, read_flag_, c_begin, p_.k };
			be_.launch(c_end - c_begin, fc, "precommit");
		}
		CommitEnv<NW> e;
		e.read_flag = read_flag_;
		e.p = p_; e.b = b; e.vis32 = (uint32_t*)vis_; e.both32 = (uint32_t*)both_;
		e.cand_read = cand_d; e.status = status_d; e.first_rec = first_d;
		e.recs = recs_; e.pool = pool_; e.result = result_d;
		e.kh = kh_; e.rkh = rkh_; e.rkoff = rkoff_d;
		e.cend = cend_; e.st = cstate_;
		e.order = order_; e.order_n = order_n_;
		be_.template launch_commit<NW>(e, c_begin, c_end);
		be_.d2h(&cs, cstate_, sizeof cs);
		counters_ = cs.counters;
		cend_count_ = cs.cend_count;
		if (cs.pad_) fail_now(FAIL_INTERNAL, "contigEndKmers table overflowed");
		return cs.break_at;
	}

	template <int NW>
	uint32_t commit_par(const Batch& b, uint32_t* cand_d, uint32_t* status_d, uint32_t* first_d,
	    uint8_t* result_d, uint64_t* rkoff_d, uint32_t c_begin, uint32_t c_end)
	{
		uint32_t n = c_end - c_begin;
		const uint32_t n0 = n;
		uint32_t nrec = 0, nord = 0;
		be_.d2h(&nrec, rec_used_, 4);
		be_.d2h(&nord, order_n_, 4);
		nrec = std::min(nrec, rec_cap_);
		{
			uint64_t need = cend_count_ + 2ull * (nrec - std::min(nord, rec_cap_));
			while (need * 2 > cend_.mask + 1) grow_cend();
		}
		const bool part = dist();
		uint8_t* part_buf = part ? (uint8_t*)be_.alloc((uint64_t)n + nrec + 64) : nullptr;
		uint8_t* part_c = part_buf; uint8_t* part_r = part ? part_buf + n : nullptr;
		uint32_t* nfirst = part ? nullptr : (uint32_t*)be_.alloc(n * 4ull + 4);
		if (nfirst) be_.memset(nfirst, 0, n * 4ull);
		{
			if (part) be_.memset(part_buf, 1, (uint64_t)n + nrec);
			FPreCommit<NW> f{ p_, b, cand_d, status_d, first_d, recs_, vis_, kh_, rkh_, rkoff_d, read_flag_, c_begin,
// ... 123 lines not shown
		}
		{ FPcBreak f{ e }; be_.launch(n, f, "pc_break"); }
		be_.d2h(scal_h, e.scal, sizeof scal_h);
		const uint32_t brk = std::min(scal_h[1], c_end);
		e.brk = brk;
		if (sliced_) {
			ParCommit ea = e; ea.cnt8 = nullptr;
			{ FPcApply f{ ea }; be_.launch_wave(n, f, "pc_apply"); }
			const uint64_t ext = g_pool_ + 64;
			uint8_t* kmin = (uint8_t*)be_.alloc(ext);
			be_.memset(kmin, 0xFF, ext);
			{ FPcCover f{ e, kmin, 0u }; be_.launch_wave(n, f, "pc_cover"); }
			c_all_reduce(kmin, g_pool_, DT_U8, OP_MIN);
			{ FPcCover f{ e, kmin, 1u }; be_.launch_wave(n, f, "pc_cover"); }
			be_.free(kmin);
		} else { FPcApply f{ e }; be_.launch_wave(n, f, "pc_apply"); }
		if (nshort) { FPcShort f{ e, 1 }; be_.launch(1, f, "pc_short"); }
		std::vector<uint64_t> c3(n);
		std::vector<uint8_t> act(n);
		be_.d2h(c1.data(), e.cnt, n * 4ull);
		be_.d2h(c2.data(), e.cnt2, n * 4ull);
		be_.d2h(c3.data(), e.cnt3, n * 8ull);
		be_.d2h(act.data(), e.active, n);
		be_.d2h(scal_h, e.scal, sizeof scal_h);
		if (scal_h[4]) fail_now(FAIL_INTERNAL, "contigEndKmers table overflowed");
		uint32_t orec = 0; uint64_t oid = 0, bases = 0, visited = 0;
		for (uint32_t i = 0; i < n && c_begin + i < brk; i++) {
			uint32_t r = c1[i], q = c2[i];
			c1[i] = orec; c2[i] = (uint32_t)oid;
			orec += r; oid += q; bases += c3[i];
			if (!act[i]) visited++;
		}
		be_.h2d(e.cnt, c1.data(), n * 4ull);
		be_.h2d(e.cnt2, c2.data(), n * 4ull);
		{ FPcWrite f{ e, order_, nord, counters_.contig_id }; be_.launch(n, f, "pc_write"); }
		nord += orec;
		be_.h2d(order_n_, &nord, 4);
		counters_.contig_id += oid;
		counters_.bases_assembled += bases;
		counters_.visited_reads += visited;
		stats_.generated += (brk - c_begin) - visited;
		cend_count_ += scal_h[3];
		if (nshort) { free_tab(e.tcend); be_.free(e.short_keys); }
		be_.free(e.off); be_.free(e.cnt); be_.free(e.cnt2); be_.free(e.cnt3); be_.free(e.active);
		be_.free(e.short_list); be_.free(e.scal);
		if (nfirst) {
			std::vector<uint32_t> nf(n);
			be_.d2h(nf.data(), nfirst, n * 4ull);
			for (uint32_t v : nf) stats_.commit_first_chunk_decided += v;
			be_.free(nfirst);
		}
		if (dirty_buf) be_.free(dirty_buf);
		if (part_buf) be_.free(part_buf);
		return brk;
	}

	void merge_walk_results(const uint32_t* list_d, uint32_t nlist, uint32_t* status_d, uint32_t* first_d, uint32_t nc)
	{
		const uint32_t R = (uint32_t)comm_.world, me = (uint32_t)comm_.rank;
		uint32_t lr = 0; uint64_t lp = 0;
		be_.d2h(&lr, rec_used_, 4);
		be_.d2h(&lp, pool_used_, 8);
		lr = std::min(lr, rec_cap_); lp = std::min<uint64_t>(lp, pool_cap_);
		std::vector<uint64_t> cnt(2 * R, 0);
		cnt[2 * me] = lr - g_rec_; cnt[2 * me + 1] = lp - g_pool_;
		host_all_reduce_sum(cnt.data(), 2 * R);
		FRecFix fx;
		fx.rbase[0] = 0; fx.pbase[0] = 0;
		for (uint32_t q = 0; q < R; q++) {
			fx.rbase[q + 1] = fx.rbase[q] + (uint32_t)cnt[2 * q];
			fx.pbase[q + 1] = fx.pbase[q] + cnt[2 * q + 1];
		}
		const uint64_t tot_rec = fx.rbase[R], tot_pool = fx.pbase[R];
		if (g_rec_ + tot_rec > rec_cap_) {
			uint32_t cap = rec_cap_;
			while (g_rec_ + tot_rec > cap) cap *= 2;
			recs_ = (ContigRec*)regrow(recs_, (uint64_t)rec_cap_ * sizeof(ContigRec), (uint64_t)cap * sizeof(ContigRec));
			order_ = (uint32_t*)regrow(order_, (uint64_t)rec_cap_ * 4, (uint64_t)cap * 4);
			rec_cap_ = cap;
		}
		if (g_pool_ + tot_pool > pool_cap_) {
			uint64_t cap = pool_cap_;
			while (g_pool_ + tot_pool > cap) cap *= 2;
			pool_ = (uint8_t*)regrow(pool_, pool_cap_, cap);
			kh_ = (uint64_t*)regrow(kh_, pool_cap_ * 8, cap * 8);
			pool_cap_ = cap;
		}
		if (me && cnt[2 * me]) {
			void* tmp = be_.alloc(cnt[2 * me] * sizeof(ContigRec));
			be_.d2d(tmp, recs_ + g_rec_, cnt[2 * me] * sizeof(ContigRec));
			be_.d2d(recs_ + g_rec_ + fx.rbase[me], tmp, cnt[2 * me] * sizeof(ContigRec));
			be_.free(tmp);
		}
		if (me && cnt[2 * me + 1]) {
			void* tmp = be_.alloc(cnt[2 * me + 1] * 8);
			be_.d2d(tmp, pool_ + g_pool_, cnt[2 * me + 1]);
			be_.d2d(pool_ + g_pool_ + fx.pbase[me], tmp, cnt[2 * me + 1]);
			be_.d2d(tmp, kh_ + g_pool_, cnt[2 * me + 1] * 8);
			be_.d2d(kh_ + g_pool_ + fx.pbase[me], tmp, cnt[2 * me + 1] * 8);
			be_.free(tmp);
		}
		std::vector<uint64_t> c(R), d(R);
		for (uint32_t q = 0; q < R; q++) { c[q] = cnt[2 * q] * sizeof(ContigRec); d[q] = (uint64_t)(g_rec_ + fx.rbase[q]) * sizeof(ContigRec); }
		if (tot_rec) c_all_gather_v(recs_, c.data(), d.data());
		for (uint32_t q = 0; q < R; q++) { c[q] = cnt[2 * q + 1]; d[q] = g_pool_ + fx.pbase[q]; }
		if (tot_pool) c_all_gather_v(pool_, c.data(), d.data());
		for (uint32_t q = 0; q < R; q++) { c[q] *= 8; d[q] *= 8; }
		if (tot_pool) c_all_gather_v(kh_, c.data(), d.data());
		if (tot_rec) {
			fx.recs = recs_; fx.g_rec = g_rec_; fx.world = R;
			be_.launch(tot_rec, fx, "merge_fix");
		}
		if (nlist && fx.rbase[me]) { FFirstFix f{ list_d, first_d, fx.rbase[me] }; be_.launch(nlist, f, "merge_fix"); }
		c_all_reduce(status_d, nc, DT_U32, OP_MAX);
		c_all_reduce(first_d, nc, DT_U32, OP_MIN);
		g_rec_ += (uint32_t)tot_rec; g_pool_ += tot_pool;
		be_.h2d(rec_used_, &g_rec_, 4);
		be_.h2d(pool_used_, &g_pool_, 8);
	}
	void* regrow(void* old, uint64_t old_bytes, uint64_t new_bytes)
	{
		void* n = be_.alloc(new_bytes);
		be_.d2d(n, old, old_bytes);
		be_.free(old);
		return n;
	}

	template <int NW>
	void prep_new_records(uint32_t& prepped)
	{
		uint32_t nrec = 0;
		be_.d2h(&nrec, rec_used_, 4);
		nrec = std::min(nrec, rec_cap_);
		if (nrec > prepped) {
			FContigPrep<NW> f{ p_, cnt_, recs_, prepped, pool_, kh_, use_par_commit() ? 0u : 1u };
			be_.launch_wave(nrec - prepped, f, "contig_prep");
			if (use_par_commit()) link_duplicates(prepped, nrec);
			prepped = nrec;
		}
	}
	void link_duplicates(uint32_t first_new, uint32_t nrec)
	{
		if (!cfg_.link_duplicates || dist() || nrec <= first_new || nrec < 2) return;
		uint64_t* key = (uint64_t*)be_.alloc(nrec * 16ull); uint64_t* key2 = key + nrec;
		uint32_t* val = (uint32_t*)be_.alloc(nrec * 8ull); uint32_t* val2 = val + nrec;
		{ FDupKeys f{ recs_, p_.k, key, val }; be_.launch(nrec, f, "dup_link"); }
		be_.sort_pairs_u64_u32(key, key2, val, val2, nrec);
		{ FDupLink f{ recs_, key2, val2, nrec, first_new }; be_.launch(nrec, f, "dup_link"); }
		{ FDupVerify f{ recs_, kh_, p_.k, first_new }; be_.launch_wave(nrec - first_new, f, "dup_link"); }
		be_.sync();
		be_.free(key); be_.free(val);
	}
	template <int NW>
	void prep_local_records()
	{
		uint32_t lr = 0;
		be_.d2h(&lr, rec_used_, 4);
		lr = std::min(lr, rec_cap_);
		if (lr > g_rec_) {
			FContigPrep<NW> f{ p_, cnt_, recs_, g_rec_, pool_, kh_, use_par_commit() ? 0u : 1u };
			be_.launch_wave(lr - g_rec_, f, "contig_prep");
		}
	}
	void grow_cend()
	{
		uint32_t log2 = 1;
		while ((1ull << log2) < cend_.mask + 1) log2++;
		WalkTab bigger{};
		alloc_tab(bigger, log2 + 2);
		uint32_t* failed = (uint32_t*)be_.alloc(8);
		be_.memset(failed, 0, 4);
		FRehash f{ cend_, bigger, failed };
		be_.launch(cend_.mask + 1, f, "rehash");
		uint32_t bad = 0;
		be_.d2h(&bad, failed, 4);
		be_.free(failed);
		if (bad) fail_now(FAIL_INTERNAL, "contigEndKmers rehash failed");
		free_tab(cend_);
		cend_ = bigger;
	}
	void ensure_wtab(uint64_t nwalk)
	{
		const uint64_t want = 2 * nwalk * wtab_per_walker_;
		uint32_t log2 = wtab_log2_;
		while ((1ull << log2) < want && log2 < wtab_log2_cap()) log2++;
		if (log2 == wtab_log2_) return;
		free_tab(wtab_);
		wtab_log2_ = log2;
		alloc_tab(wtab_, wtab_log2_);
		if (cfg_.verbose) fprintf(stderr, "abyss_amd: walker vertex table grown to 2^%u entries\n", wtab_log2_);
	}
	uint32_t wtab_log2_cap()
	{
		uint32_t cap = cfg_.wtab_log2_max;
		const uint64_t mem = be_.device_mem_bytes();
		while (mem && cap > cfg_.wtab_log2 && (24ull << cap) > mem / 8) cap--;
		return cap;
	}
	void clear_wtab()
	{
		be_.memset(wtab_.hmin, 0xFF, (wtab_.mask + 1) * 8);
		be_.memset(wtab_.meta, 0xFF, (wtab_.mask + 1) * 8);
	}

	struct BatchRun {
		Batch v{};
		uint64_t first = 0, n = 0;
		uint8_t* res_d = nullptr;
		std::vector<uint32_t> cand_h;
		uint32_t nc = 0;
		uint32_t* cand_d = nullptr; uint32_t* status_d = nullptr; uint32_t* first_d = nullptr;
		uint32_t* need_d = nullptr; uint32_t* need_n = nullptr; uint64_t* rkoff_d = nullptr;
		uint32_t base = 0;
		uint32_t prepped = 0, owner_next = 0, committed = 0, force = 0xFFFFFFFFu, nneed = 0, nneed_all = 0;
		bool round_started = false;
		bool predicted = false;
		bool pending = false;
		bool overflow = false, debug = false;
	};
	template <int NW>
	void assemble_nw(const Batch& b, uint8_t* result_d, uint8_t* results_host,
	    const std::function<void(const ContigOut&)>& sink)
	{
		uint64_t next = 0;
		while (next < b.n) {
			ensure_walk();
			BatchRun r;
			classify_batch<NW>(b, next, std::min<uint64_t>(p2_batch_, b.n - next), result_d, r);
			next += r.n;
			counters_.reads_processed += r.n;
			p2_batch_ = next_batch_size();
			prefetch_ = nullptr;
// ... 151 lines not shown
		prep_new_records<NW>(r.prepped);
		r.committed = base; r.force = 0xFFFFFFFFu; r.overflow = false;
		r.round_started = true;
		predict_and_walk<NW>(r);
	}
	template <int NW>
	void predict_and_walk(BatchRun& r)
	{
		const uint32_t nc = r.nc;
		be_.memset(r.need_n, 0, 8);
		{
			FPredict<NW> fp{ p_, r.v, r.cand_d, r.status_d, vis_, r.rkoff_d, rkh_,
				r.need_d, r.need_n, r.committed, r.force, (uint32_t)comm_.rank, (uint32_t)comm_.world };
			be_.launch(nc - r.committed, fp, "predict");
		}
		uint32_t nn2[2] = { 0, 0 };
		be_.d2h(nn2, r.need_n, 8);
		r.nneed = nn2[0];
		r.nneed_all = comm_.world > 1 ? nn2[1] : r.nneed;
		r.predicted = true; r.pending = false;
		if (!r.nneed_all) return;
		if (r.owner_next > 0xF0000000u - nc) { r.overflow = true; return; }
		ensure_wtab(std::max<uint32_t>(r.nneed, 1));
		clear_wtab();
		WalkEnv<NW> env = make_env<NW>(r.v, r.cand_d, r.status_d, r.first_d);
		env.owner_base = r.owner_next;
		r.owner_next += nc;
		FWalk<NW> fw{ env, r.need_d };
		if (prefetch_) { prefetch_(); prefetch_ = nullptr; }
		be_.launch_walkers(r.nneed, fw, wslots_, "rewalk");
		r.pending = true;
	}

	template <int NW>
	void finish_batch(BatchRun& r, const std::function<void(const ContigOut&)>& sink)
	{
		const uint32_t nc = r.nc;
		while (r.base < nc) {
			if (!r.round_started) start_round<NW>(r);
			while (r.committed < nc && !r.overflow) {
				if (!r.predicted) predict_and_walk<NW>(r);
				r.predicted = false;
				if (r.overflow) break;
				if (r.pending) {
					r.pending = false;
					stats_.rewalked += r.nneed_all;
					dump_walkers(r, "rewalk", r.nneed);
					if (dist()) {
						prep_local_records<NW>();
						merge_walk_results(r.need_d, r.nneed, r.status_d, r.first_d, nc);
						r.prepped = g_rec_;
					} else prep_new_records<NW>(r.prepped);
				}
				uint32_t next = use_par_commit() ? commit_par<NW>(r.v, r.cand_d, r.status_d, r.first_d, r.res_d, r.rkoff_d, r.committed, nc)
				                                 : commit<NW>(r.v, r.cand_d, r.status_d, r.first_d, r.res_d, r.rkoff_d, r.committed, nc);
				if (next < nc) {
					stats_.breaks++;
					uint32_t st = 0;
					be_.d2h(&st, r.status_d + next, 4);
					if (st == WS_OVERFLOW) { r.committed = next; r.overflow = true; break; }
					if (next == r.committed && (st == WS_COMPLETE || r.force == next)) {
						fail_now(FAIL_INTERNAL, strf("commit made no progress at candidate %llu (status %llu)", next, st));
					}
					r.force = next;
				}
				r.committed = next;
			}
			deliver(r.cand_h, r.first, sink);
			if (r.overflow) {
				stats_.overflows++;
				uint64_t pool_now = 0; uint32_t recs_now = 0;
				be_.d2h(&pool_now, pool_used_, 8);
				be_.d2h(&recs_now, rec_used_, 4);
				bool pool_out = pool_now > pool_cap_, recs_out = recs_now > rec_cap_;
				if (dist()) {
					uint64_t ovf[2] = { 0, 0 };
					be_.d2h(ovf, wstats_ + WSTAT_OVF_POOL, 16);
					pool_out = pool_out || ovf[0] != ovf_seen_[0]; recs_out = recs_out || ovf[1] != ovf_seen_[1];
					ovf_seen_[0] = ovf[0]; ovf_seen_[1] = ovf[1];
				}
				if (pool_out) {
					be_.free(pool_); be_.free(kh_);
					pool_cap_ *= 2;
					pool_ = (uint8_t*)be_.alloc(pool_cap_);
					kh_ = (uint64_t*)be_.alloc(pool_cap_ * 8);
					if (cfg_.verbose) fprintf(stderr, "abyss_amd: contig pool grown to %llu bases\n", (unsigned long long)pool_cap_);
				}
				if (recs_out) {
					be_.free(recs_); be_.free(order_);
					rec_cap_ *= 2;
					recs_ = (ContigRec*)be_.alloc((uint64_t)rec_cap_ * sizeof(ContigRec));
					order_ = (uint32_t*)be_.alloc((uint64_t)rec_cap_ * 4);
					if (cfg_.verbose) fprintf(stderr, "abyss_amd: contig records grown to %u\n", rec_cap_);
				}
				if (!pool_out && !recs_out) {
					if (r.committed == r.base) grow_walk_resources();
					else wtab_per_walker_ *= 2;
				}
			}
			r.base = r.committed;
			r.round_started = false; r.predicted = false; r.pending = false;
		}
		be_.free(rkh_); rkh_ = nullptr;
		be_.free(read_flag_); read_flag_ = nullptr;
		if (r.debug) { be_.free(dbg_); dbg_ = nullptr; }
		be_.free(r.cand_d); be_.free(r.status_d); be_.free(r.first_d);
		be_.free(r.need_d); be_.free(r.need_n); be_.free(r.rkoff_d);
		r.cand_h.clear();
	}

	void deliver(const std::vector<uint32_t>& cand_h, uint64_t read_base,
	    const std::function<void(const ContigOut&)>& sink)
	{
		if (!sink) return;
		uint32_t n = 0;
		be_.d2h(&n, order_n_, 4);
		if (!n) return;
		std::vector<uint32_t> order(n);
		be_.d2h(order.data(), order_, n * 4ull);
		uint32_t nrec = 0;
		be_.d2h(&nrec, rec_used_, 4);
		nrec = std::min(nrec, rec_cap_);
		std::vector<ContigRec> recs(nrec);
		be_.d2h(recs.data(), recs_, nrec * sizeof(ContigRec));
		uint64_t used = 0;
		be_.d2h(&used, pool_used_, 8);
		used = std::min<uint64_t>(used, pool_cap_);
		std::vector<uint8_t> pool(used);
		be_.d2h(pool.data(), pool_, used);
		deliveries_wait();
		const std::function<void(const ContigOut&)>* sk = &sink;
		delivery_ = std::async(std::launch::async,
		    [sk, read_base, n, order = std::move(order), recs = std::move(recs), pool = std::move(pool), cand = cand_h]() {
			ContigOut o;
			for (uint32_t i = 0; i < n; i++) {
				const ContigRec& r = recs[order[i]];
				o.contig_id = r.redundant ? ~0ULL : r.contig_id;
				o.read_index = read_base + cand[r.cand];
				o.seq.resize(r.len);
				for (uint32_t j = 0; j < r.len; j++) o.seq[j] = "ACGTN"[pool[r.seq_off + j] <= 4 ? pool[r.seq_off + j] : 4];
				o.coverage = r.redundant ? 0 : r.coverage;
				o.redundant = r.redundant != 0;
				o.left_ext = r.left_ext; o.right_ext = r.right_ext;
				o.left_code = r.left_code; o.right_code = r.right_code;
				o.seed_pos = r.seed_pos;
				(*sk)(o);
			}
		});
	}
	std::future<void> delivery_;
	void deliveries_wait() { if (delivery_.valid()) delivery_.get(); }

};

}
```

abyss_amd/csrc/abg_host.h:

```cpp
#pragma once
#include "abg_engine.h"
#include "../../include/abyss_amd.h"

#include <cctype>
#include <cmath>
#include <map>
#include <string>
#include <atomic>
#include <chrono>
#include <future>
#include <memory>
#include <thread>

namespace abg {
static_assert(FAIL_NOMEM == ABG_ENOMEM && FAIL_INTERNAL == ABG_EINTERNAL, "Failure codes are the C ABI's");


struct FContainsSolid {
	Params p; const uint64_t* h0; const uint8_t* cnt; uint8_t* out;
	ABG_HD void operator()(uint64_t t, uint32_t) const { out[t] = solid_contains(p, cnt, h0[t]) ? 1 : 0; }
};
struct FExpand {
	Params p; const uint64_t* h0; uint64_t* out;
	ABG_HD void operator()(uint64_t t, uint32_t) const
	{
		uint64_t h = h0[t];
		for (unsigned i = 0; i < p.nh; i++) out[t * p.nh + i] = hash_i(p, h, i);
	}
};

inline uint64_t counters_for_budget(uint64_t bloom_bytes)
{
	double sz = (double)bloom_bytes / 1.125 / 1.0;
	uint64_t n = (uint64_t)std::round(sz);
	uint64_t rem = n % 64;
	return rem ? n + 64 - rem : n;
}

template <class BE>
class Session {
  public:
	std::string error;
	BE be;
	Engine<BE>* eng = nullptr;
	Config cfg;

	template <class... A>
	explicit Session(A&&... a) : be(std::forward<A>(a)...) {}
	~Session() { try { drain(); } catch (...) {} keep_drop(false); delete eng; }

	int create(const abg_params& p)
	{
		if (p.k < 2 || p.k > ABG_MAX_KMER) return fail(ABG_EINVAL, "k must be in 2.." + std::to_string(ABG_MAX_KMER));
		if (p.num_hashes < 1 || p.num_hashes > ABG_MAX_HASHES) return fail(ABG_EINVAL, "num_hashes must be in 1..32");
		if (p.spaced_seed && p.spaced_seed[0]) {
			std::string m(p.spaced_seed);
			if (m.size() != p.k) return fail(ABG_EINVAL, "spaced seed must be exactly k bits long");
			if (m.find_first_not_of("01") != std::string::npos) return fail(ABG_EINVAL, "spaced seed must contain only '0's or '1's");
			if (m.front() != '1' || m.back() != '1') return fail(ABG_EINVAL, "spaced seed must begin and end with '1's");
			if (!std::equal(m.begin(), m.end(), m.rbegin())) return fail(ABG_EINVAL, "spaced seed must be symmetric");
			if (m.find('0') != std::string::npos) cfg.spaced_seed = m;
		}
		cfg.k = p.k; cfg.nh = p.num_hashes; cfg.kc = p.min_cov;
		cfg.trim = (p.trim == 0xFFFFFFFFu) ? p.k : p.trim;
		cfg.counters = p.counters ? p.counters : counters_for_budget(p.bloom_bytes);
		cfg.cascade_levels = p.cascade_levels;
		cfg.slice_filter = p.slice_filter;
		if (const char* e = getenv("ABG_SLICE_FILTER")) cfg.slice_filter = (uint32_t)atoi(e);
		if (p.cascade_levels && (!p.counters || p.counters % 64)) return fail(ABG_EINVAL, "cascade mode needs `counters` = bits per level, a multiple of 64");
		if (!cfg.counters) return fail(ABG_EINVAL, "bloom_bytes / counters must be > 0");
		cfg.verbose = p.verbose;
		if (p.insert_batch_kmers) cfg.insert_batch_kmers = p.insert_batch_kmers;
		if (p.claim_log2) cfg.claim_log2 = p.claim_log2;
		if (p.walk_slots) cfg.walk_slots = p.walk_slots;
		if (p.wtab_log2) cfg.wtab_log2 = p.wtab_log2;
		if (const char* e = getenv("ABG_CLAIM_LOG2")) cfg.claim_log2 = (uint32_t)atoi(e);
		if (const char* e = getenv("ABG_INSERT_BATCH")) cfg.insert_batch_kmers = strtoull(e, 0, 10);
		if (const char* e = getenv("ABG_WALK_SLOTS")) cfg.walk_slots = (uint32_t)atoi(e);
		if (const char* e = getenv("ABG_WTAB_LOG2")) cfg.wtab_log2 = (uint32_t)atoi(e);
		if (const char* e = getenv("ABG_WTAB_LOG2_MAX")) cfg.wtab_log2_max = (uint32_t)std::max<int>(atoi(e), (int)cfg.wtab_log2);
		if (const char* e = getenv("ABG_POOL_CAP")) cfg.pool_cap = std::max<uint64_t>(1024, strtoull(e, 0, 10));
		if (const char* e = getenv("ABG_REC_CAP")) cfg.rec_cap = (uint32_t)std::max(16, atoi(e));
		if (const char* e = getenv("ABG_P2_FIRST_BATCH")) cfg.p2_first_batch = strtoull(e, 0, 10);
		if (const char* e = getenv("ABG_P2_MAX_BATCH")) cfg.p2_max_batch = strtoull(e, 0, 10);
		if (const char* e = getenv("ABG_PAR_COMMIT")) cfg.par_commit = atoi(e) != 0;
		if (const char* e = getenv("ABG_T_TAGS")) cfg.t_tags = (uint32_t)std::max(2, atoi(e));
		if (const char* e = getenv("ABG_COMMIT_INCREMENTAL")) cfg.commit_incremental = (uint32_t)std::min(2, std::max(0, atoi(e)));
		if (const char* e = getenv("ABG_COMMIT_DIRTY_MAX")) cfg.commit_dirty_max = (uint32_t)std::max(0, atoi(e));
		if (const char* e = getenv("ABG_COMMIT_DIRTY_LOG2")) cfg.commit_dirty_log2 = (uint32_t)std::min(34, std::max(10, atoi(e)));
		if (const char* e = getenv("ABG_PAR_COMMIT_MAX_GB")) cfg.par_commit_max_bytes = strtoull(e, 0, 10) << 30;
		if (const char* e = getenv("ABG_COMPACT_THRESHOLD")) cfg.compact_threshold = strtoull(e, 0, 10);
		if (const char* e = getenv("ABG_TILED")) cfg.tiled_insert = atoi(e) != 0;
		if (const char* e = getenv("ABG_DIST_ROUTE_MIN")) cfg.dist_route_min_ranks = (uint32_t)atoi(e);
		if (const char* e = getenv("ABG_BENIGN")) cfg.benign_sharers = atoi(e) != 0;
		if (const char* e = getenv("ABG_CLS_ARCHIVE")) cfg.cls_archive = atoi(e) != 0;
		if (const char* e = getenv("ABG_CLS_DEBUG_SKIP")) cfg.cls_debug_skip = (uint32_t)atoi(e);
		if (const char* e = getenv("ABG_CLS_ARCHIVE_MAX_MB")) cfg.cls_archive_max_mb = (uint32_t)std::max(0, atoi(e));
		if (const char* e = getenv("ABG_SORTED_OVERFLOW")) cfg.sorted_overflow = atoi(e) != 0;
		if (const char* e = getenv("ABG_COSETTLE")) cfg.cosettle = atoi(e) != 0;
		if (const char* e = getenv("ABG_CLS_BOTH")) cfg.cls_both = atoi(e) != 0;
		if (const char* e = getenv("ABG_CLS_BOTH_MAX_MB")) cfg.cls_both_max_mb = (uint32_t)std::max(0, atoi(e));
		if (const char* e = getenv("ABG_COSETTLE_PASSES")) cfg.cosettle_passes = (uint32_t)std::max(1, atoi(e));
		if (const char* e = getenv("ABG_COSETTLE_LOG2")) cfg.cosettle_log2 = (uint32_t)std::min(25, std::max(5, atoi(e)));
		if (const char* e = getenv("ABG_LINK_DUPS")) cfg.link_duplicates = atoi(e) != 0;
		if (const char* e = getenv("ABG_OVERLAP_PURITY")) cfg.overlap_purity = atoi(e) != 0;
		if (const char* e = getenv("ABG_LEAD_IMPLICIT")) cfg.lead_implicit = atoi(e) != 0;
		if (const char* e = getenv("ABG_APPLY_MASK")) cfg.apply_mask = atoi(e) != 0;
		if (const char* e = getenv("ABG_OVERLAP_BINS")) cfg.overlap_bins = atoi(e) != 0;
		if (const char* e = getenv("ABG_PREFETCH")) cfg.prefetch_classify = atoi(e) != 0;
		if (const char* e = getenv("ABG_ASYNC_LOAD")) cfg.async_load = atoi(e) != 0;
		if (const char* e = getenv("ABG_CLS_SLOTS")) cfg.classify_slots = (uint32_t)std::max(64, atoi(e));
		if (const char* e = getenv("ABG_SOLID_PLANE")) cfg.solid_plane = atoi(e) != 0;
		if (const char* e = getenv("ABG_MEMO")) cfg.memo = atoi(e) != 0;
		if (const char* e = getenv("ABG_P2_MAX_CANDIDATES")) cfg.p2_max_candidates = (uint32_t)std::max(1, atoi(e));
		if (const char* e = getenv("ABG_P2_STARVED_GROWTH")) cfg.p2_starved_growth = (uint32_t)std::max(2, atoi(e));
		if (const char* e = getenv("ABG_P2_STARVED")) cfg.p2_starved = (uint32_t)atoi(e);
		if (const char* e = getenv("ABG_P2_GROWTH")) cfg.p2_growth = (uint32_t)std::max(2, atoi(e));
		if (const char* e = getenv("ABG_DRAIN_THRESHOLD")) cfg.drain_threshold = (uint32_t)strtoul(e, 0, 10);
		if (const char* e = getenv("ABG_GUIDE_STRIDE")) cfg.guide_stride = (uint32_t)strtoul(e, 0, 10);
		if (const char* e = getenv("ABG_GUIDE_SEEN")) cfg.guide_seen = atoi(e) != 0;
		if (const char* e = getenv("ABG_GUIDE_LOG2_MAX")) cfg.guide_log2_max = (uint32_t)std::min(36, std::max(10, atoi(e)));
		if (!be.ok()) return fail(ABG_ENODEV, be.why());
		eng = new Engine<BE>(be, cfg);
		return ABG_OK;
	}

	int load_seqs(const char* seqs, const uint64_t* off, uint64_t n) { return load_seqs_v(1, &seqs, &off, &n); }
	int load_seqs_v(uint32_t nchunks, const char* const* seqs_v, const uint64_t* const* off_v, const uint64_t* n_v)
	{
		const uint32_t k = cfg.k;
		const double t_call = std::chrono::duration<double>(std::chrono::steady_clock::now().time_since_epoch()).count();
		const uint32_t max_piece = (uint32_t)std::min<uint64_t>(1u << 20, cfg.insert_batch_kmers + k - 1);
		struct Part { uint32_t c; uint64_t a, b; };
		std::vector<Part> plan;
		std::vector<uint64_t> base(nchunks + 1, 0);
		for (uint32_t c = 0; c < nchunks; c++) {
			base[c + 1] = base[c] + n_v[c];
			if (!n_v[c]) continue;
			const std::vector<uint64_t> cut = split_reads(off_v[c], n_v[c]);
			for (size_t t = 0; t + 1 < cut.size(); t++) plan.push_back(Part{ c, cut[t], cut[t + 1] });
		}
		const bool keeping = keep_on_ && !keep_failed_;
		std::vector<KeptPart> kparts(keeping ? plan.size() : 0);
		std::vector<uint8_t> verdict(keeping ? base[nchunks] : 0, (uint8_t)RR_UNINITIALIZED);
		std::vector<HostBatch> parts(plan.size());
		const bool timing = getenv("ABG_HOST_TIMING") != nullptr;
		const auto tnow = []() { return std::chrono::duration<double>(std::chrono::steady_clock::now().time_since_epoch()).count(); };
		const double t0 = tnow();
		run_parts(parts.size(), [&](size_t t) {
			HostBatch& hb = parts[t];
			const Part& pt = plan[t];
			const char* seqs = seqs_v[pt.c];
			const uint64_t* off = off_v[pt.c];
			{
				const uint64_t nr = pt.b - pt.a, bases = off[pt.b] - off[pt.a];
				hb.words.reserve(bases / 16 + nr + 1); hb.woff.reserve(nr + 1); hb.len.reserve(nr); hb.koff.reserve(nr + 1);
				if (keeping) { kparts[t].read.reserve(nr); kparts[t].piece.reserve(nr); kparts[t].len.reserve(nr); }
			}
			std::string up;
			std::vector<std::pair<uint64_t, uint64_t>> runs;
			std::vector<uint8_t> bad;
			for (uint64_t i = pt.a; i < pt.b; i++) {
				const char* s = seqs + off[i];
				uint64_t L = off[i + 1] - off[i];
				if (L < k) { if (keeping) verdict[base[pt.c] + i] = (uint8_t)RR_SHORTER_THAN_K; continue; }
				const char* text = s;
				if (!cfg.spaced_seed.empty()) {
					up.assign(s, L);
					for (auto& ch : up) ch = (char)toupper((unsigned char)ch);
					text = up.data();
				}
				bool clean = false;
				if (keeping) {
					uint8_t any = 0;
					for (uint64_t q = 0; q < L; q++) any |= codes_.t[(unsigned char)s[q]];
					clean = !(any & 0x80);
					if (!clean) verdict[base[pt.c] + i] = (uint8_t)RR_NON_ACGT;
				}
				if (clean && L <= max_piece) {
					kparts[t].read.push_back(base[pt.c] + i); kparts[t].piece.push_back(hb.n()); kparts[t].len.push_back((uint32_t)L);
					hb.add_ascii(text, (uint32_t)L, k);
					continue;
				}
				if (clean) { kparts[t].extra.add_ascii(text, (uint32_t)L, k); kparts[t].extra_read.push_back(base[pt.c] + i); }
				valid_runs(text, L, runs, bad);
				for (auto& run : runs) {
					uint64_t pa = run.first, pb = run.second - 1 + k;
// ... 687 lines not shown
```

abyss_amd/csrc/abg_kernels.hip:

```cpp
#include <hip/hip_runtime.h>
#include <hip/hip_ext.h>
#include <hipcub/hipcub.hpp>
#include <rccl/rccl.h>
#include <dlfcn.h>
#include <unistd.h>

#include "abg_host.h"
#include "abg_overlap.h"

#include <chrono>
#include <map>
#include <mutex>

namespace {

template <class F>
__global__ void __launch_bounds__(256) k_foreach(F f, uint64_t n)
{
	uint64_t i = (uint64_t)blockIdx.x * blockDim.x + threadIdx.x;
	const uint64_t stride = (uint64_t)gridDim.x * blockDim.x;
	const uint32_t slot = (uint32_t)i;
	for (; i < n; i += stride) f(i, slot);
}
#ifndef ABG_CLS_WAVES
// ... 1024 lines not shown
	if (!ctx || !out) return ABG_EINVAL;
	return guarded(ctx, [&]() -> int {
		*out = ctx->s.be.try_alloc(bytes);
		if (!*out) { ctx->s.error = "device allocation failed"; return ABG_ENOMEM; }
		return ABG_OK;
	});
}
int abg_dev_free(abg_ctx* ctx, void* ptr)
{
	if (!ctx) return ABG_EINVAL;
	return guarded(ctx, [&]() -> int {
		if (ptr) { ctx->s.be.sync(); hipFree(ptr); }
		return ABG_OK;
	});
}
int abg_dev_copy(abg_ctx* ctx, void* dst, const void* src, uint64_t n, int32_t kind)
{
	if (!ctx || (n && (!dst || !src)) || kind < 0 || kind > 2) return ABG_EINVAL;
	return guarded(ctx, [&]() -> int {
		if (kind == 0) ctx->s.be.h2d(dst, src, n);
		else if (kind == 1) ctx->s.be.d2h(dst, src, n);
		else { ctx->s.be.d2d(dst, src, n); ctx->s.be.sync(); }
		return ABG_OK;
	});
}
int abg_output_graph_seqs(abg_ctx* ctx, const char* seqs, const uint64_t* offsets, uint64_t n,
    abg_text_cb cb, void* user, uint64_t* nodes, uint64_t* edges)
{
	if (!ctx || (n && (!seqs || !offsets))) return ABG_EINVAL;
	return guarded(ctx, [&]() -> int {
		return ctx->s.output_graph_seqs(seqs, offsets, n, cb, user, nodes, edges);
	});
}
int abg_profile_enable(abg_ctx* ctx, int on)
{
	if (!ctx) return ABG_EINVAL;
	return guarded(ctx, [&]() -> int {
		ctx->s.be.prof_drain();
		ctx->s.be.profiling = on != 0;
		return ABG_OK;
	});
}
int abg_profile_reset(abg_ctx* ctx)
{
	if (!ctx) return ABG_EINVAL;
	return guarded(ctx, [&]() -> int {
		ctx->s.be.prof_drain(true);
		ctx->s.be.prof.clear();
		return ABG_OK;
	});
}
int abg_profile_get(abg_ctx* ctx, const char* name, double* total_ms, uint64_t* launches)
{
	if (!ctx || !name) return ABG_EINVAL;
	return guarded(ctx, [&]() -> int {
		ctx->s.be.prof_drain();
		auto it = ctx->s.be.prof.find(name);
		double ms = 0;
		uint64_t n = 0;
		if (it != ctx->s.be.prof.end()) { ms = it->second.ms; n = it->second.launches; }
		if (total_ms) *total_ms = ms;
		if (launches) *launches = n;
		return ABG_OK;
	});
}
int abg_get_stats(const abg_ctx* ctx, abg_stats* out)
{
	if (!ctx || !out) return ABG_EINVAL;
	return guarded((abg_ctx*)ctx, [&]() -> int {
		auto s = ctx->s.eng->stats();
		out->insert_rounds = s.insert_rounds;
		out->walk_rounds = s.rounds;
		out->candidates = s.candidates;
		out->walked = s.walked;
		out->rewalked = s.rewalked;
		out->commit_breaks = s.breaks; out->commit_rounds = s.commit_rounds; out->generated = s.generated;
		out->bulk_calls = s.bulk_calls; out->bulk_steps = s.bulk_steps; out->lin_steps = s.lin_steps; out->guide_slots = s.guide_slots; out->chain_steps = s.chain_steps; out->batch_cuts = s.batch_cuts; out->overflows = s.overflows;
		out->memo_hits = s.memo_hits; out->memo_adds = s.memo_adds;
		out->tiled_ops = s.tiled_ops; out->tiled_pending = s.tiled_pending; out->tile_overflows = s.tile_overflows;
		out->cls_covered_reads = s.cls_covered_reads; out->archive_bases = s.archive_bases; out->cls_decided_reads = s.cls_decided_reads;
		out->counter_bytes_held = ctx->s.eng->counter_bytes_held();
		out->commit_rounds_incremental = s.commit_rounds_incremental; out->commit_dirty_records = s.commit_dirty_records;
		out->commit_first_chunk_decided = s.commit_first_chunk_decided;
		return ABG_OK;
	});
}

}
struct abg_overlap {
	HipBackend be;
	abg::OverlapJoin<HipBackend> join;
	std::string error;
	explicit abg_overlap(int dev) : be(dev), join(be) {}
};
namespace {
std::string g_overlap_create_error;
template <class F>
int guarded_ov(abg_overlap* o, F&& body)
{
	try {
		return body();
	} catch (const abg::Failure& f) {
		o->error = f.msg;
		return f.code;
	} catch (const std::bad_alloc&) {
		o->error = "host memory exhausted";
		return ABG_ENOMEM;
	} catch (const std::exception& e) {
		o->error = e.what();
		return ABG_EINTERNAL;
	}
}
}
extern "C" {
int abg_overlap_create(int device, abg_overlap** out)
{
	if (!out) return ABG_EINVAL;
	*out = nullptr;
	abg_overlap* o = nullptr;
	try {
		o = new abg_overlap(device);
	} catch (const std::exception& e) {
		g_overlap_create_error = e.what();
		return ABG_EINTERNAL;
	}
	if (!o->be.ok()) {
		g_overlap_create_error = o->be.why();
		delete o;
		return ABG_ENODEV;
	}
	*out = o;
	return ABG_OK;
}
void abg_overlap_destroy(abg_overlap* o) { delete o; }
const char* abg_overlap_last_error(const abg_overlap* o) { return o ? o->error.c_str() : g_overlap_create_error.c_str(); }
int abg_overlap_join(abg_overlap* o, uint32_t overlap, uint64_t n_contigs, const uint64_t* head_keys, const uint64_t* tail_keys,
    int strand_specific, uint64_t* n_edges)
{
	if (!o || !n_edges || (n_contigs && (!head_keys || !tail_keys))) return ABG_EINVAL;
	if (overlap < 1 || overlap > 32 * abg::OV_MAX_WORDS) { o->error = "overlap length out of range (1..256)"; return ABG_EINVAL; }
	if (n_contigs >= (1ull << 30)) { o->error = "too many contigs (vertex ids are 32-bit)"; return ABG_EINVAL; }
	return guarded_ov(o, [&]() -> int {
		o->join.run(overlap, n_contigs, head_keys, tail_keys, strand_specific != 0);
		*n_edges = o->join.edges();
		return ABG_OK;
	});
}
int abg_overlap_edges(abg_overlap* o, uint64_t* offsets, uint32_t* targets)
{
	if (!o) return ABG_EINVAL;
	return guarded_ov(o, [&]() -> int {
		o->join.fetch(offsets, targets);
		return ABG_OK;
	});
}
int abg_overlap_profile(abg_overlap* o, int on)
{
	if (!o) return ABG_EINVAL;
	o->be.prof_drain();
	o->be.profiling = on != 0;
	return ABG_OK;
}
int abg_overlap_profile_get(abg_overlap* o, const char* name, double* total_ms, uint64_t* launches)
{
	if (!o || !name) return ABG_EINVAL;
	o->be.prof_drain();
// ... 8 lines not shown
```

abyss_amd/csrc/abg_walk.h:

```cpp
#pragma once
#include "abg_core.h"

namespace abg {

struct Batch {
	const uint32_t* words;
	const uint64_t* woff;
	const uint32_t* len;
	const uint64_t* koff;
	uint64_t n;
};
ABG_HD unsigned batch_base(const Batch& b, uint64_t r, uint32_t i)
{
	uint32_t w = b.words[b.woff[r] + (i >> 4)];
	return (w >> (2 * (i & 15))) & 3u;
}
template <int NW>
ABG_HD Kmer<NW> batch_kmer(const Batch& b, uint64_t r, uint32_t pos, unsigned k)
{
	return window_kmer<NW>(b.words, b.woff[r], pos, k);
}
ABG_HD uint64_t find_seq(const uint64_t* koff, uint64_t n, uint64_t t)
{
	uint64_t lo = 0, hi = n;
// ... 5 lines not shown
}

constexpr uint64_t WT_EMPTY = ~0ULL;
constexpr uint32_t WT_TOMB = 0xFFFFFFFEu;
struct WalkTab {
	uint64_t* hmin;
	uint64_t* hmax;
	uint64_t* meta;
	uint64_t mask;
};
ABG_HD VKey wt_key(VKey key)
{
	if (key.fh == WT_EMPTY) key.fh = WT_EMPTY - 1;
	return key;
}
template <int NW>
ABG_HD VKey vtx_key(const Params& p, const Vtx<NW>& v) { return wt_key(vtx_ident(p, v)); }
ABG_HD uint64_t wt_slot(const WalkTab& t, const VKey& key, uint32_t owner)
{
	uint64_t x = key.fh ^ ((uint64_t)(owner + 1) * 0xD6E8FEB86659FD93ULL);
	x ^= x >> 32; x *= 0xD6E8FEB86659FD93ULL; x ^= x >> 29;
	return x & t.mask;
}
enum { WT_NEW = 0, WT_SAME_CONTIG = 1, WT_EARLIER = 2, WT_FULL = 3 };
ABG_HD int wt_insert(const WalkTab& t, const VKey& key, uint32_t owner, uint32_t contig, bool coop = false)
{
	uint64_t s = wt_slot(t, key, owner);
	for (uint64_t probes = 0; probes <= t.mask; probes++, s = (s + 1) & t.mask) {
		uint64_t cur = wu_cas_u64(&t.hmin[s], WT_EMPTY, key.fh, coop);
		if (cur == WT_EMPTY) {
			wu_st_coherent(&t.hmax[s], key.rh, coop);
			wu_st_coherent(&t.meta[s], ((uint64_t)owner << 32) | contig, coop);
			return WT_NEW;
		}
		if (cur != key.fh) continue;
		uint64_t m = ld_coherent(&t.meta[s]);
		if ((uint32_t)(m >> 32) != owner) continue;
		if (ld_coherent(&t.hmax[s]) != key.rh) continue;
		uint32_t c = (uint32_t)m;
		if (c == contig) return WT_SAME_CONTIG;
		wu_st_coherent(&t.meta[s], ((uint64_t)owner << 32) | contig, coop);
		return c == WT_TOMB ? WT_NEW : WT_EARLIER;
	}
	return WT_FULL;
}
ABG_HD uint64_t wt_find(const WalkTab& t, const VKey& key, uint32_t owner)
{
	uint64_t s = wt_slot(t, key, owner);
	for (uint64_t probes = 0; probes <= t.mask; probes++, s = (s + 1) & t.mask) {
		uint64_t cur = ld_coherent(&t.hmin[s]);
		if (cur == WT_EMPTY) return WT_EMPTY;
		if (cur != key.fh) continue;
		uint64_t m = ld_coherent(&t.meta[s]);
		if ((uint32_t)(m >> 32) != owner) continue;
		if (ld_coherent(&t.hmax[s]) != key.rh) continue;
		return s;
	}
	return WT_EMPTY;
}


enum WalkStatus : uint32_t {
	WS_NONE = 0,
	WS_COMPLETE = 1,
	WS_OVERFLOW = 3
};
struct ContigRec {
	uint64_t seq_off;
	uint32_t len;
	uint32_t cand;
	uint32_t next;
	uint32_t seed_pos;
	uint32_t left_ext, right_ext;
	uint8_t left_code, right_code;
	uint8_t redundant;
	uint8_t pre_redundant;
	uint32_t coverage;
	uint64_t contig_id;
	uint32_t time;
	uint32_t ins;
	uint32_t ins_prev;
	uint32_t dup_of;
	uint64_t fp;
};
constexpr uint32_t REC_END = 0xFFFFFFFFu;

template <int NW>
struct WalkEnv {
	Params p;
	const uint8_t* cnt;
	Batch batch;
	const uint32_t* cand_read;
	uint32_t* status;
	uint32_t* first_rec;
	WalkTab tab;
	uint32_t owner_base;
	TBFrame<NW>* tb_pool; VKey* tbk_pool; uint32_t tb_cap;
	void* fast; uint32_t fast_bytes;
	VKey* la_pool;
	uint8_t* lbuf_pool; uint8_t* rbuf_pool; uint32_t buf_cap;
	uint64_t* dbg;
	bool coop;
	Guide guide;
	SuccMemo memo;
	MaskCache* mcache;
	BulkScratch* bulk_pool;
	uint64_t* wstats;
	uint8_t* pool; uint64_t pool_cap; uint64_t* pool_used;
	ContigRec* recs; uint32_t rec_cap; uint32_t* rec_used;
};

template <int NW>
struct WalkState {
	Vtx<NW> seed;
	uint8_t* lbuf; uint8_t* rbuf;
	uint32_t nl, nr;
	Vtx<NW> head;
	VKey prev_key;
	uint32_t ext;
	int32_t ins;
	BulkScratch* bulk;
	uint32_t bulk_skip;
	uint32_t bulk_overflow;
	uint32_t n_bulk_calls, n_bulk_steps, n_lin_steps;
	uint32_t n_bulk_tries;
	uint64_t t_bx[6];
	uint64_t t_seed, t_ext, t_mat;
	uint64_t t_bulk, t_lin, t_post;
	uint64_t t_bp[4];
};
template <int NW>
ABG_HD unsigned ws_base(const Params& p, const WalkState<NW>& w, uint32_t j)
{
	if (j < w.nl) return w.lbuf[w.nl - 1 - j];
	j -= w.nl;
	if (j < p.k) return kmer_get(w.seed.s, j);
	return w.rbuf[j - p.k];
}
template <int NW>
ABG_HDN Vtx<NW> ws_vertex(const Params& p, const WalkState<NW>& w, uint32_t i, bool coop = false)
{
	return gather_vertex<NW>(p, coop, [&](unsigned j) { return ws_base(p, w, i + j); });
}
template <int NW>
ABG_HDN Vtx<NW> pool_vertex(const Params& p, const uint8_t* seq, uint64_t i, bool coop = false)
{
	return gather_vertex<NW>(p, coop, [&](unsigned j) { return (unsigned)seq[i + j] & 3u; });
}

ABG_HD uint64_t dbg_clock(const uint64_t* dbg)
{
#if defined(__HIP_DEVICE_COMPILE__)
	return dbg ? wall_clock64() : 0;
#else
	(void)dbg; return 0;
#endif
}
template <int NW, bool COOP>
ABG_HDX uint32_t walk_bulk(const WalkEnv<NW>& e, WalkState<NW>& w, const int dir_in, const uint32_t owner_in,
    const uint32_t contig_in, const uint64_t hint_in)
{
	{
	const uint64_t tq0 = dbg_clock(e.dbg);
	const Params p = uniform_params<COOP>(e.p);
	const unsigned k = p.k;
	const uint8_t* __restrict__ cnt = uniptr<COOP>(e.cnt);
// ... 646 lines not shown
		if (lcode < 0) break;
		int rcode = walk_extend(e, w, FORWARD, owner, contig, sc, &rext, &abort_status, &right_earlier);
		if (rcode < 0) break;
		uint32_t n = w.nl + 1 + w.nr;
		total_steps += n;
		const uint64_t tp0 = dbg_clock(e.dbg);
		if (e.dbg) w.t_ext += tp0 - te0;

		const bool tip = is_tip(n, lcode, rcode, p.trim);
		if (!tip) {
			uint64_t need = (uint64_t)n + k - 1 + 2;
			uint64_t off = wu_atomic_add_u64(e.pool_used, need, sc.coop);
			if (off + need > e.pool_cap) {
				wu_atomic_add_u64(&e.wstats[WSTAT_OVF_POOL], 1, sc.coop);
				abort_status = WS_OVERFLOW; break;
			}
			uint8_t* S = e.pool + off + 1;
			uint64_t slen = (uint64_t)n + k - 1;
			for (uint64_t j = sc.coop ? lane_id() : 0u; j < slen; j += sc.coop ? 64u : 1u) S[j] = (uint8_t)ws_base(p, w, (uint32_t)j);
			wave_sync();
			int64_t lo = 0, hi = (int64_t)n;
			Vtx<NW> popped[2]; bool popped_earlier[2]; int npopped = 0;
			Vtx<NW> pushed; int pushed_side = 0;
			if (n > 1) {
				Vtx<NW> front = pool_vertex<NW>(p, S, 0, sc.coop), back = pool_vertex<NW>(p, S, n - 1, sc.coop);
				int type = CT_LINEAR;
				{
					uint64_t nfh[4], nrh[4];
					unsigned mask = neighbour_mask(p, e.cnt, back, SENSE, nfh, nrh, sc.coop);
					bool edge = false;
					for (unsigned b = 0; b < 4; b++) {
						if (!((mask >> b) & 1u)) continue;
						Vtx<NW> x = make_neighbour(p, back, SENSE, b, nfh[b], nrh[b]);
						if (vtx_equal(p, x, front)) { edge = true; break; }
					}
					if (edge) {
						Vtx<NW> x = front;
						vtx_shift(p, x, ANTISENSE, kmer_get(back.s, 0));
						type = kmer_equal(p, x.s, back.s) ? CT_CIRCULAR : CT_HAIRPIN;
					}
				}
				if (type != CT_LINEAR && n > 2) {
					bool bstart = ambiguous1(p, e.cnt, front, FORWARD, sc) || ambiguous1(p, e.cnt, front, REVERSE, sc);
					bool bend = ambiguous1(p, e.cnt, back, FORWARD, sc) || ambiguous1(p, e.cnt, back, REVERSE, sc);
					if (bstart && !bend) {
						unsigned nb = (type == CT_CIRCULAR) ? kmer_get(front.s, k - 1) : 3u - kmer_get(front.s, 0);
						S[hi + k - 1] = (uint8_t)nb;
						hi++;
						pushed = front; pushed_side = 1;
						if (type != CT_CIRCULAR) vtx_revcomp(p, pushed);
					} else if (!bstart && bend) {
						unsigned nb = (type == CT_CIRCULAR) ? kmer_get(back.s, 0) : 3u - kmer_get(back.s, k - 1);
						S[lo - 1] = (uint8_t)nb;
						lo--;
						pushed = back; pushed_side = -1;
						if (type != CT_CIRCULAR) vtx_revcomp(p, pushed);
					}
				}
				int64_t l = hi - lo;
				Vtx<NW> p0 = pool_vertex<NW>(p, S, lo, sc.coop), p1 = pool_vertex<NW>(p, S, lo + 1, sc.coop);
				Vtx<NW> q1 = pool_vertex<NW>(p, S, hi - 1, sc.coop), q2 = pool_vertex<NW>(p, S, hi - 2, sc.coop);
				if (pushed_side > 0) q1 = pushed;
				if (pushed_side < 0) p0 = pushed;
				(void)l;
				bool amb1 = ambiguous2(p, e.cnt, p0, p1, FORWARD, sc);
				bool amb2 = ambiguous2(p, e.cnt, q1, q2, REVERSE, sc);
				if (amb1) { popped[npopped] = p0; popped_earlier[npopped] = (lo == 0) ? (w.nl ? left_earlier : seed_earlier) : true; npopped++; lo++; }
				if (amb2) { popped[npopped] = q1; popped_earlier[npopped] = (hi == (int64_t)n) ? (w.nr ? right_earlier : seed_earlier) : true; npopped++; hi--; }
				if ((pushed_side < 0 && amb1) || (pushed_side > 0 && amb2)) pushed_side = 0;
			}
			if (sc.overflow) { abort_status = WS_OVERFLOW; break; }
			uint32_t ri = wu_atomic_add_u32(e.rec_used, 1, sc.coop);
			if (ri >= e.rec_cap) {
				wu_atomic_add_u64(&e.wstats[WSTAT_OVF_RECS], 1, sc.coop);
				abort_status = WS_OVERFLOW; break;
			}
			ContigRec& rec = e.recs[ri];
			rec.seq_off = off + 1 + (uint64_t)lo;
			rec.len = (uint32_t)(hi - lo) + k - 1;
			rec.cand = c; rec.next = REC_END; rec.seed_pos = it;
			rec.left_ext = lext; rec.right_ext = rext;
			rec.left_code = (uint8_t)lcode; rec.right_code = (uint8_t)rcode;
			rec.redundant = 0; rec.pre_redundant = 0; rec.coverage = 0; rec.contig_id = ~0ULL;
			rec.ins_prev = 0; rec.dup_of = REC_END; rec.fp = 0;
			if (last == REC_END) first = ri; else e.recs[last].next = ri;
			last = ri;
			if (npopped) {
				Vtx<NW> nf = pool_vertex<NW>(p, S, lo, sc.coop), nb = pool_vertex<NW>(p, S, hi - 1, sc.coop);
				if (pushed_side < 0) nf = pushed;
				if (pushed_side > 0) nb = pushed;
				for (int q = 0; q < npopped; q++) {
					if (popped_earlier[q]) continue;
					if (hi > lo && (vtx_equal(p, popped[q], nf) || vtx_equal(p, popped[q], nb))) continue;
					uint64_t s = wt_find(e.tab, vtx_key(p, popped[q]), owner);
					if (s != WT_EMPTY) wu_st_coherent(&e.tab.meta[s], ((uint64_t)owner << 32) | WT_TOMB, sc.coop);
				}
			}
			if (p.mask && hi > lo && (uint64_t)(hi - lo) < k) {
				const MaskTab& m = *p.mask;
				const uint32_t np = (uint32_t)(hi - lo);
				uint8_t* C = S + lo;
				for (uint32_t col = np; col + 1 < k; col++) {
					uint32_t j0 = col - np + 1, j1 = col + 1;
					if (m.ones_prefix[j1] == m.ones_prefix[j0]) C[col] = 4;
				}
			}
		}
		contig++;
		if (e.dbg) { ts0 = dbg_clock(e.dbg); w.t_post += ts0 - tp0; }
	}
	e.first_rec[c] = first;
	e.status[c] = abort_status ? abort_status : (uint32_t)WS_COMPLETE;
	if (e.wstats) {
		wu_atomic_add_u64(&e.wstats[WSTAT_BULK_CALLS], w.n_bulk_calls, sc.coop);
		wu_atomic_add_u64(&e.wstats[WSTAT_BULK_STEPS], w.n_bulk_steps, sc.coop);
		wu_atomic_add_u64(&e.wstats[WSTAT_LIN_STEPS], w.n_lin_steps, sc.coop);
		wu_atomic_add_u64(&e.wstats[WSTAT_CHAIN_STEPS], sc.n_chain_steps, sc.coop);
		wu_atomic_add_u64(&e.wstats[WSTAT_MEMO_HITS], sc.n_memo_hits, sc.coop);
		wu_atomic_add_u64(&e.wstats[WSTAT_MEMO_ADDS], sc.n_memo_adds, sc.coop);
	}
	if (e.dbg) {
#if defined(__HIP_DEVICE_COMPILE__)
		const uint64_t t_end = wall_clock64();
#else
		const uint64_t t_end = 0;
#endif
		uint64_t* d = e.dbg + (uint64_t)c * WALK_DBG_N;
		d[0] = t_end - t_start; d[1] = total_steps; d[2] = sc.dbg_search; d[3] = sc.dbg_calls;
		d[4] = sc.dbg_nodes; d[5] = w.t_bulk; d[6] = contig; d[7] = w.t_post;
		d[8] = w.t_lin; d[9] = w.n_bulk_tries; d[10] = w.n_bulk_calls; d[11] = w.n_bulk_steps; d[12] = sc.dbg_chain;
		d[13] = sc.dbg_la; d[14] = sc.dbg_la_calls; d[15] = w.t_bp[1]; d[16] = sc.dbg_mask; d[17] = sc.dbg_mask_n; d[18] = sc.dbg_memo;
		d[19] = w.t_seed + (dbg_clock(e.dbg) - ts0); d[20] = w.t_ext; d[21] = w.t_mat;
		for (int q = 0; q < 6; q++) d[22 + q] = w.t_bx[q];
	}
}

ABG_HD unsigned code_rank(unsigned c) { return c == 4 ? 3u : (c == 3 ? 4u : c); }
ABG_HD unsigned code_comp(unsigned c) { return c == 4 ? 4u : 3u - c; }
ABG_HDN VKey canonical_end_key(const Params& p, const uint8_t* seq)
{
	const unsigned k = p.k;
	bool rc_less = false;
	for (unsigned i = 0; i < k; i++) {
		unsigned a = code_rank(code_comp(seq[k - 1 - i])), b = code_rank(seq[i]);
		if (a != b) { rc_less = a < b; break; }
	}
	auto text = [&](unsigned i) -> unsigned { return rc_less ? code_comp(seq[k - 1 - i]) : (unsigned)seq[i]; };
	uint64_t fs, rs;
	scratch_hashes(p, text, fs, rs);
	VKey key;
	if (p.ident_fast) {
		key.fh = rs < fs ? rs : fs;
		key.rh = rs < fs ? fs : rs;
		return wt_key(key);
	}
	bool canon = true;
	for (unsigned i = 0; i < k / 2; i++) {
		unsigned c1 = code_rank(text(i)), c2 = code_rank(code_comp(text(k - 1 - i)));
		if (c1 > c2) { canon = false; break; }
		if (c1 < c2) break;
	}
	key.fh = canon ? fs : rs;
	key.rh = canon ? rs : fs;
	return wt_key(key);
}

}
// ... 1 lines not shown
```

include/abyss_amd.h:

```cpp
#ifndef ABYSS_AMD_H
#define ABYSS_AMD_H 1

#include <stddef.h>
#include <stdint.h>

#ifdef __cplusplus
extern "C" {
#endif

#define ABG_OK 0
#define ABG_EINVAL (-1)
#define ABG_ENODEV (-2)
#define ABG_ENOMEM (-3)
#define ABG_EINTERNAL (-4)
#define ABG_EAGAIN (-5)

#define ABG_MAX_KMER 192
#define ABG_MAX_HASHES 32

enum abg_read_result {
	ABG_RR_UNINITIALIZED = 0,
	ABG_RR_SHORTER_THAN_K,
	ABG_RR_NON_ACGT,
	ABG_RR_BLUNT_END,
// ... 70 lines not shown
    const uint32_t* d_len, uint64_t n);

int abg_counting_stats(abg_ctx* ctx, uint64_t* popcount, uint64_t* filtered_popcount);

int abg_counters_export(abg_ctx* ctx, uint8_t* host_out);
int abg_counters_import(abg_ctx* ctx, const uint8_t* host_in);
int abg_visited_export(abg_ctx* ctx, uint8_t* host_out);
int abg_visited_import(abg_ctx* ctx, const uint8_t* host_in);

int abg_assemble_seqs(abg_ctx* ctx, const char* seqs, const uint64_t* offsets, uint64_t n,
    uint8_t* results, abg_contig_cb cb, void* user);
int abg_assemble_seqs_v(abg_ctx* ctx, uint32_t nchunks, const char* const* seqs, const uint64_t* const* offsets,
    const uint64_t* n, uint8_t* results, abg_contig_cb cb, void* user);
int abg_assemble_packed(abg_ctx* ctx, const uint32_t* d_words, const uint64_t* d_woff,
    const uint32_t* d_len, uint64_t n, uint8_t* results, abg_contig_cb cb, void* user);

int abg_cascade_export(abg_ctx* ctx, uint32_t level, uint8_t* host_out);

int abg_get_counters(const abg_ctx* ctx, abg_counters* out);
int abg_set_counters(abg_ctx* ctx, const abg_counters* in);

int abg_hash_seq(abg_ctx* ctx, const char* seq, uint64_t len, uint32_t* pos_out,
    uint64_t* hashes_out, uint64_t cap, uint64_t* n_out);

int abg_contains_seq(abg_ctx* ctx, const char* seq, uint64_t len, uint32_t* pos_out,
    uint8_t* contains_out, uint64_t cap, uint64_t* n_out);

enum abg_dtype { ABG_U8 = 0, ABG_U32 = 1, ABG_U64 = 2 };
enum abg_redop { ABG_SUM = 0, ABG_MAX = 1, ABG_MIN = 2 };
typedef struct abg_comm {
	int32_t rank, world;
	int32_t stream_ordered;
	int32_t struct_size;
	void* user;
	int (*all_gather_v)(void* user, void* buf, const uint64_t* counts, const uint64_t* displs, void* stream);
	int (*all_reduce)(void* user, void* buf, uint64_t count, int32_t dtype, int32_t op, void* stream);
	int (*all_to_all_v)(void* user, const void* send, const uint64_t* send_counts, const uint64_t* send_displs,
	    void* recv, const uint64_t* recv_counts, const uint64_t* recv_displs, void* stream);
} abg_comm;
#define ABG_MAX_RANKS 16

int abg_attach_comm(abg_ctx* ctx, const abg_comm* comm);

int abg_share_reads(abg_ctx* ctx, const uint32_t* d_words, const uint64_t* d_woff, const uint32_t* d_len,
    uint64_t n_local, const uint32_t** g_words, const uint64_t** g_woff, const uint32_t** g_len,
    uint64_t* n_total);

int abg_rccl_unique_id(uint8_t id[128]);
int abg_rccl_comm_create(const uint8_t id[128], int32_t rank, int32_t world, int32_t device, abg_comm* out);
int abg_rccl_comm_destroy(abg_comm* comm);

int abg_dev_copy(abg_ctx* ctx, void* dst, const void* src, uint64_t n, int32_t kind);
int abg_dev_alloc(abg_ctx* ctx, uint64_t bytes, void** out);
int abg_dev_free(abg_ctx* ctx, void* ptr);

typedef void (*abg_text_cb)(void* user, const char* text, uint64_t len);
int abg_output_graph_seqs(abg_ctx* ctx, const char* seqs, const uint64_t* offsets, uint64_t n,
    abg_text_cb cb, void* user, uint64_t* nodes, uint64_t* edges);

int abg_profile_enable(abg_ctx* ctx, int on);
int abg_profile_reset(abg_ctx* ctx);
int abg_profile_get(abg_ctx* ctx, const char* name, double* total_ms, uint64_t* launches);
typedef struct abg_stats {
	uint64_t insert_rounds, walk_rounds, candidates, walked, rewalked, commit_breaks;
	uint64_t commit_rounds;
	uint64_t generated;
	uint64_t bulk_calls, bulk_steps;
	uint64_t lin_steps;
	uint64_t guide_slots;
	uint64_t chain_steps;
	uint64_t batch_cuts;
	uint64_t overflows;
	uint64_t memo_hits, memo_adds;
	uint64_t tiled_ops;
	uint64_t tiled_pending;
	uint64_t tile_overflows;
	uint64_t cls_covered_reads;
	uint64_t archive_bases;
	uint64_t cls_decided_reads;
	uint64_t counter_bytes_held;
	uint64_t commit_rounds_incremental;
	uint64_t commit_dirty_records;
	uint64_t commit_first_chunk_decided;
} abg_stats;
int abg_get_stats(const abg_ctx* ctx, abg_stats* out);

typedef struct abg_overlap abg_overlap;
int abg_overlap_create(int device, abg_overlap** out);
void abg_overlap_destroy(abg_overlap* o);
const char* abg_overlap_last_error(const abg_overlap* o);
int abg_overlap_join(abg_overlap* o, uint32_t overlap, uint64_t n_contigs, const uint64_t* head_keys,
    const uint64_t* tail_keys, int strand_specific, uint64_t* n_edges);
int abg_overlap_edges(abg_overlap* o, uint64_t* offsets, uint32_t* targets);
int abg_overlap_profile(abg_overlap* o, int on);
int abg_overlap_profile_get(abg_overlap* o, const char* name, double* total_ms, uint64_t* launches);

typedef struct abg_rr abg_rr;
int abg_rr_create(int device, uint64_t bytes, uint32_t hash_num, uint32_t r, abg_rr** out);
void abg_rr_destroy(abg_rr* f);
const char* abg_rr_last_error(const abg_rr* f);
int abg_rr_bytes(const abg_rr* f, uint64_t* bytes);
int abg_rr_clear(abg_rr* f);
int abg_rr_insert_seqs(abg_rr* f, const char* seqs, const uint64_t* offsets, uint64_t n, uint32_t max_bases,
    const uint32_t* lengths, uint32_t n_lengths, uint64_t* n_inserted);
int abg_rr_contains_seqs(abg_rr* f, const char* seqs, const uint64_t* offsets, uint64_t n, uint32_t* found);
int abg_rr_popcount(abg_rr* f, uint64_t* bits_set);
int abg_rr_export(abg_rr* f, uint8_t* host_out);
int abg_rr_sync(abg_rr* f);
int abg_rr_profile(abg_rr* f, int on);
int abg_rr_profile_get(abg_rr* f, const char* name, double* total_ms, uint64_t* launches);


typedef struct abg_kn abg_kn;
int abg_kn_create(int device, uint64_t full_bits, uint32_t levels, uint32_t k, uint64_t seed, uint64_t start, uint64_t end,
    abg_kn** out);
void abg_kn_destroy(abg_kn* f);
const char* abg_kn_last_error(const abg_kn* f);
int abg_kn_import(abg_kn* f, uint32_t level, const uint8_t* bytes);
int abg_kn_export(abg_kn* f, uint32_t level, uint8_t* bytes);
int abg_kn_insert_seqs(abg_kn* f, const char* seqs, const uint64_t* offsets, uint64_t n);
int abg_kn_contains_seqs(abg_kn* f, const char* seqs, const uint64_t* offsets, uint64_t n, int inverse, uint8_t* print);
int abg_kn_popcount(abg_kn* f, uint64_t* per_level);
int abg_kn_hash_seq(abg_kn* f, const char* seq, uint64_t len, uint64_t* hash, uint64_t* index, uint8_t* valid);
int abg_kn_sync(abg_kn* f);
int abg_kn_profile(abg_kn* f, int on);
int abg_kn_profile_get(abg_kn* f, const char* name, double* total_ms, uint64_t* launches);

typedef struct abg_fm abg_fm;
typedef struct abg_fm_hit { uint32_t l, u, qstart, qend, num, pos; } abg_fm_hit;
#define ABG_FM_NO_RC 1u
#define ABG_FM_SS 2u
int abg_fm_create(int device, abg_fm** out);
void abg_fm_destroy(abg_fm* f);
const char* abg_fm_last_error(const abg_fm* f);
int abg_fm_build(abg_fm* f, const uint8_t* text, uint64_t n);
int abg_fm_size(const abg_fm* f, uint64_t* n);
int abg_fm_export(abg_fm* f, uint32_t* sa, uint8_t* bwt);
int abg_fm_map_seqs(abg_fm* f, const char* seqs, const uint64_t* offsets, uint64_t n, uint32_t min_len, uint32_t flags,
    abg_fm_hit* out);
int abg_fm_sync(abg_fm* f);
int abg_fm_tune(abg_fm* f, uint32_t waves_per_cu);
int abg_fm_profile(abg_fm* f, int on);
int abg_fm_profile_get(abg_fm* f, const char* name, double* total_ms, uint64_t* launches);

typedef struct abg_de abg_de;
typedef struct abg_de_job { int32_t first, last; uint32_t len0, len1; } abg_de_job;
typedef struct abg_de_pair { int32_t first, last; uint32_t len0, len1, l, rf; } abg_de_pair;
int abg_de_create(int device, abg_de** out);
void abg_de_destroy(abg_de* d);
const char* abg_de_last_error(const abg_de* d);
int abg_de_set_pmf(abg_de* d, const double* pmf, uint64_t n, double minp, double mean);
int abg_de_scan(abg_de* d, const abg_de_job* jobs, uint64_t njobs, const int32_t* sample_values, const uint32_t* sample_counts,
    const uint64_t* offsets, double* c, double* like, uint32_t* n);
int abg_de_estimate(abg_de* d, const abg_de_pair* pairs, uint64_t npairs, const int32_t* samples, const uint64_t* offsets,
    int32_t* distance, uint32_t* num_pairs);
int abg_de_tune(abg_de* d, uint32_t block_threads);
int abg_de_profile(abg_de* d, int on);
int abg_de_profile_get(abg_de* d, const char* name, double* total_ms, uint64_t* launches);

typedef struct abg_ov abg_ov;
typedef struct abg_ov_pair { uint32_t t, h; } abg_ov_pair;
enum { ABG_OV_TOP = 0, ABG_OV_ALL = 1 };
int abg_ov_create(int device, abg_ov** out);
void abg_ov_destroy(abg_ov* o);
const char* abg_ov_last_error(const abg_ov* o);
int abg_ov_set_contigs(abg_ov* o, const uint8_t* bytes, const uint64_t* offsets, uint64_t n);
// ... 46 lines not shown
```

Baseline: 1677.

## Link duplicate contigs from bases and copy their k-mer hashes instead of rehashing

```diff
diff --git a/abyss_amd/_lib.py b/abyss_amd/_lib.py
--- a/abyss_amd/_lib.py
+++ b/abyss_amd/_lib.py
@@ -37,7 +37,8 @@
     _fields_ = [(n, C.c_uint64) for n in
                 ("insert_rounds", "walk_rounds", "candidates", "walked", "rewalked", "commit_breaks",
                  "commit_rounds", "generated", "bulk_calls", "bulk_steps", "lin_steps", "guide_slots", "chain_steps", "batch_cuts", "overflows", "memo_hits", "memo_adds", "tiled_ops", "tiled_pending", "tile_overflows", "cls_covered_reads", "archive_bases", "cls_decided_reads", "counter_bytes_held",
-                 "commit_rounds_incremental", "commit_dirty_records", "commit_first_chunk_decided")]
+                 "commit_rounds_incremental", "commit_dirty_records", "commit_first_chunk_decided",
+                 "dup_links", "dup_links_rev", "prep_hashed_kmers", "prep_copied_kmers", "prep_chain_rehashed", "prep_copy_mismatch", "dup_scan_cut")]
 
 
 CONTIG_CB = C.CFUNCTYPE(None, C.c_void_p, C.POINTER(Contig))
diff --git a/abyss_amd/build.py b/abyss_amd/build.py
--- a/abyss_amd/build.py
+++ b/abyss_amd/build.py
@@ -129,8 +129,8 @@
 
 
 def build_hostcheck(force: bool = False) -> str:
-    src = os.path.join(ROOT, "tests", "hostcheck", "hostcheck_ext.cc")
-    if force or _newer(HOSTCHECK, [src, os.path.join(ROOT, "tests", "hostcheck", "hostcheck.cc")] + csrc_files()):
+    src = os.path.join(ROOT, "tests", "hostcheck", "hostcheck_ext2.cc")
+    if force or _newer(HOSTCHECK, [src] + [os.path.join(ROOT, "tests", "hostcheck", f) for f in ("hostcheck_ext.cc", "hostcheck.cc")] + csrc_files()):
         _run(["g++", "-std=c++17", "-O2", "-g", "-fPIC", "-shared", "-Wno-unknown-pragmas", "-o", HOSTCHECK, src])
     rsrc = os.path.join(ROOT, "tests", "hostcheck", "reader_check.cc")
     if force or _newer(READER_CHECK, [rsrc, os.path.join(CSRC, "host", "fasta_reader.h")]):
diff --git a/abyss_amd/csrc/abg_core.h b/abyss_amd/csrc/abg_core.h
--- a/abyss_amd/csrc/abg_core.h
+++ b/abyss_amd/csrc/abg_core.h
@@ -1141,6 +1141,16 @@
 }
 #else
 ABG_HD void wave_count_add(uint64_t* counter, bool want) { if (want) *counter += 1; }
+#endif
+
+#if defined(__HIP_DEVICE_COMPILE__)
+ABG_HD void wave_sum_add(uint64_t* counter, uint64_t v)
+{
+	for (int m = 32; m; m >>= 1) v += (uint64_t)__shfl_xor((unsigned long long)v, m);
+	if (v && __lane_id() == 0) atomicAdd((unsigned long long*)counter, (unsigned long long)v);
+}
+#else
+ABG_HD void wave_sum_add(uint64_t* counter, uint64_t v) { *counter += v; }
 #endif
 
 #if defined(__HIP_DEVICE_COMPILE__)
diff --git a/abyss_amd/csrc/abg_engine.h b/abyss_amd/csrc/abg_engine.h
--- a/abyss_amd/csrc/abg_engine.h
+++ b/abyss_amd/csrc/abg_engine.h
@@ -74,6 +74,8 @@
 	uint32_t guide_log2_max = 31;
 	bool guide_seen = true;
 	bool link_duplicates = true;
+	bool dup_bases = true;
+	bool prep_check = false;
 	bool par_commit = true;
 	bool overlap_bins = true;
 	bool overlap_purity = true;
@@ -1773,13 +1775,21 @@
 			    [&](uint32_t j, uint64_t h) { out[j] = h; });
 	}
 };
+ABG_HD bool dup_takes_copy(const ContigRec* recs, const ContigRec& rec, uint32_t first_new)
+{
+	const uint32_t o = rec.dup_of;
+	return o != REC_END && !(o >= first_new && recs[o].dup_of != REC_END);
+}
 template <int NW>
 struct FContigPrep {
 	Params p; const uint8_t* cnt; ContigRec* recs; uint32_t first; const uint8_t* pool; uint64_t* kh;
 	uint32_t with_cov;
+	const uint32_t* list = nullptr;
 	ABG_HDN void operator()(uint64_t i, uint32_t lane, uint32_t nlanes) const
 	{
-		ContigRec& rec = recs[first + i];
+		const bool unlinked_only = list != nullptr;
+		if (unlinked_only && i >= list[0]) return;
+		ContigRec& rec = recs[unlinked_only ? list[1 + i] : first + i];
 		const uint8_t* seq = pool + rec.seq_off;
 		uint64_t* out = kh + rec.seq_off;
 		uint32_t cnk = rec.len - p.k + 1;
@@ -1787,9 +1797,9 @@
 		uint64_t fp = 0;
 		for (uint32_t j0 = lane * PREP_RUN; j0 < cnk; j0 += nlanes * PREP_RUN)
 			kmer_hash_run(p, [&](unsigned q) { return (unsigned)seq[q]; }, j0, j0 + PREP_RUN < cnk ? j0 + PREP_RUN : cnk,
-			    [&](uint32_t j, uint64_t h) { out[j] = h; fp += dup_mix(h); if (with_cov) cov += solid_min_count(p, cnt, h); });
+			    [&](uint32_t j, uint64_t h) { out[j] = h; if (!unlinked_only) fp += dup_mix(h); if (with_cov) cov += solid_min_count(p, cnt, h); });
 		if (cov) atomic_add_u32(&rec.coverage, cov);
-		if (fp) atomic_add_u64(&rec.fp, fp);
+		if (fp && !unlinked_only) atomic_add_u64(&rec.fp, fp);
 	}
 };
 
@@ -1804,6 +1814,7 @@
 };
 struct FDupLink {
 	ContigRec* recs; const uint64_t* key; const uint32_t* val; uint64_t n; uint32_t first_new;
+	uint64_t* cut;
 	ABG_HD void operator()(uint64_t q, uint32_t) const
 	{
 		const uint32_t me = val[q];
@@ -1811,11 +1822,14 @@
 		const uint64_t k = key[q];
 		uint64_t g = q;
 		for (unsigned s = 0; s < 64 && g > 0 && key[g - 1] == k; s++) g--;
+		bool beyond = g > 0 && key[g - 1] == k;
 		uint32_t best = REC_END, best_cand = recs[me].cand;
 		for (unsigned s = 0; s < 128 && g < n && key[g] == k; s++, g++) {
 			const uint32_t o = val[g];
 			if (o != me && recs[o].cand < best_cand && recs[o].len == recs[me].len && recs[o].fp == recs[me].fp) { best = o; best_cand = recs[o].cand; }
 		}
+		beyond = beyond || (g < n && key[g] == k);
+		if (beyond) atomic_add_u64(cut, 1);
 		recs[me].dup_of = best;
 	}
 };
@@ -1832,6 +1846,160 @@
 		for (uint32_t j = lane; j < nk; j += nlanes) { const uint64_t x = a[j]; fwd = fwd & (x == b[j]); rev = rev & (x == b[nk - 1 - j]); }
 		fwd = wave_all_lanes(fwd, nlanes); rev = wave_all_lanes(rev, nlanes);
 		if (!fwd && !rev && lane == 0) d.dup_of = REC_END;
+		if (!fwd && rev && lane == 0) d.dup_rev = 1;
+	}
+};
+constexpr uint64_t POOL_PAD = 8;
+ABG_HD uint64_t pool_bytes8(const uint64_t* poolw, uint64_t wmax, uint64_t at)
+{
+	const uint64_t q = at >> 3;
+	const unsigned s = (unsigned)(at & 7) * 8;
+	const uint64_t a = poolw[q < wmax ? q : wmax], b = poolw[q + 1 < wmax ? q + 1 : wmax];
+	return s ? (a >> s) | (b << (64 - s)) : a;
+}
+ABG_HD uint64_t pack8_2bit(uint64_t w)
+{
+	w &= 0x0303030303030303ULL;
+	w = (w | (w >> 6)) & 0x000F000F000F000FULL;
+	w = (w | (w >> 12)) & 0x000000FF000000FFULL;
+	return (w | (w >> 24)) & 0xFFFFu;
+}
+ABG_HD uint64_t rev_2bit_groups(uint64_t x)
+{
+	x = ((x >> 2) & 0x3333333333333333ULL) | ((x & 0x3333333333333333ULL) << 2);
+	x = ((x >> 4) & 0x0F0F0F0F0F0F0F0FULL) | ((x & 0x0F0F0F0F0F0F0F0FULL) << 4);
+	return __builtin_bswap64(x);
+}
+ABG_HD uint64_t slice_2bit(uint64_t lo, uint64_t hi, uint32_t g)
+{
+	return g >= 32 ? hi >> (2 * (g - 32)) : g ? (lo >> (2 * g)) | (hi << (64 - 2 * g)) : lo;
+}
+constexpr uint32_t FPB_RUN = 32;
+struct FDupFp {
+	ContigRec* recs; uint32_t first; const uint64_t* poolw; uint64_t wmax; uint32_t k;
+	ABG_HDN void operator()(uint64_t i, uint32_t lane, uint32_t nlanes) const
+	{
+		ContigRec& rec = recs[first + i];
+		if (rec.len < k + FP_TRIM - 1) return;
+		const uint32_t W = k < 32 ? k : 32;
+		const uint64_t M = W < 32 ? (1ULL << (2 * W)) - 1 : ~0ULL;
+		const uint32_t nwin = rec.len - W + 1;
+		uint64_t fp = 0;
+		for (uint32_t j0 = lane * FPB_RUN; j0 < nwin; j0 += nlanes * FPB_RUN) {
+			const uint64_t at = rec.seq_off + j0, q0 = at >> 3;
+			const unsigned s = (unsigned)(at & 7) * 8;
+			uint64_t w[9];
+#pragma unroll
+			for (uint32_t q = 0; q < 9; q++) w[q] = poolw[q0 + q < wmax ? q0 + q : wmax];
+			uint64_t P0 = 0, P1 = 0;
+#pragma unroll
+			for (uint32_t q = 0; q < 8; q++) {
+				const uint64_t x = pack8_2bit(s ? (w[q] >> s) | (w[q + 1] << (64 - s)) : w[q]) << (16 * (q & 3));
+				if (q < 4) P0 |= x; else P1 |= x;
+			}
+			const uint64_t R0 = rev_2bit_groups(~P1), R1 = rev_2bit_groups(~P0);
+#pragma unroll
+			for (uint32_t q = 0; q < FPB_RUN; q++) {
+				const uint64_t f = slice_2bit(P0, P1, q) & M, r = slice_2bit(R0, R1, 64 - W - q) & M;
+				if (j0 + q < nwin) fp += dup_mix(f < r ? f : r);
+			}
+		}
+		if (fp) atomic_add_u64(&rec.fp, fp);
+	}
+};
+struct FDupVerifyBases {
+	ContigRec* recs; const uint64_t* poolw; uint64_t wmax; uint32_t first_new;
+	ABG_HDN void operator()(uint64_t i, uint32_t lane, uint32_t nlanes) const
+	{
+		ContigRec& d = recs[first_new + i];
+		const uint32_t o = d.dup_of;
+		if (o == REC_END) return;
+		const uint64_t a = d.seq_off, b = recs[o].seq_off;
+		const uint32_t len = d.len;
+		bool fwd = true, rev = true;
+		if (len < 8) {
+			const uint8_t* pool = (const uint8_t*)poolw;
+			for (uint32_t j = lane; j < len; j += nlanes) { const unsigned x = pool[a + j]; fwd = fwd & (x == pool[b + j]); rev = rev & (x == 3u - pool[b + len - 1 - j]); }
+		} else {
+			constexpr uint32_t U = 2;
+			for (uint32_t c0 = lane * 8; c0 < len; c0 += U * nlanes * 8) {
+				uint64_t x[U], f[U], r[U];
+#pragma unroll
+				for (uint32_t u = 0; u < U; u++) {
+					const uint32_t c = c0 + u * nlanes * 8, j = c + 8 <= len ? c : len - 8;
+					x[u] = pool_bytes8(poolw, wmax, a + j); f[u] = pool_bytes8(poolw, wmax, b + j); r[u] = pool_bytes8(poolw, wmax, b + (len - 8 - j));
+				}
+#pragma unroll
+				for (uint32_t u = 0; u < U; u++) { fwd = fwd & (x[u] == f[u]); rev = rev & (x[u] == (__builtin_bswap64(r[u]) ^ 0x0303030303030303ULL)); }
+			}
+		}
+		fwd = wave_all_lanes(fwd, nlanes); rev = wave_all_lanes(rev, nlanes);
+		if (lane == 0) {
+			if (!fwd && !rev) d.dup_of = REC_END;
+			else d.dup_rev = fwd ? 0 : 1;
+		}
+	}
+};
+struct FDupCopy {
+	const ContigRec* recs; uint64_t* kh; uint32_t k; uint32_t first_new;
+	ABG_HDN void operator()(uint64_t i, uint32_t lane, uint32_t nlanes) const
+	{
+		const ContigRec& d = recs[first_new + i];
+		if (!dup_takes_copy(recs, d, first_new)) return;
+		const uint64_t* in = kh + recs[d.dup_of].seq_off;
+		uint64_t* out = kh + d.seq_off;
+		const uint32_t nk = d.len - k + 1;
+		const bool rev = d.dup_rev != 0;
+		constexpr uint32_t U = 4;
+		for (uint32_t j0 = lane; j0 < nk; j0 += U * nlanes) {
+			uint64_t v[U];
+#pragma unroll
+			for (uint32_t u = 0; u < U; u++) {
+				const uint32_t j = j0 + u * nlanes < nk ? j0 + u * nlanes : nk - 1;
+				v[u] = in[rev ? nk - 1 - j : j];
+			}
+#pragma unroll
+			for (uint32_t u = 0; u < U; u++) if (j0 + u * nlanes < nk) out[j0 + u * nlanes] = v[u];
+		}
+	}
+};
+enum : uint32_t { PSTAT_LINKS = 0, PSTAT_LINKS_REV, PSTAT_HASHED, PSTAT_COPIED, PSTAT_CHAIN, PSTAT_MISMATCH, PSTAT_CUT, PSTAT_N };
+struct FPrepList {
+	const ContigRec* recs; uint32_t k; uint32_t first_new, nrec; uint32_t* list; uint64_t* st;
+	ABG_HDN void operator()(uint64_t i, uint32_t lane, uint32_t nlanes) const
+	{
+		uint64_t links = 0, links_rev = 0, chain = 0, hashed = 0, copied = 0;
+		for (uint32_t q = 0; q < 64; q += nlanes) {
+			const uint64_t ri = first_new + i * 64 + q + lane;
+			const bool in = ri < nrec;
+			const ContigRec& r = recs[in ? ri : first_new];
+			const bool linked = in && r.dup_of != REC_END, copy = in && list && dup_takes_copy(recs, r, first_new);
+			links += linked ? 1 : 0; links_rev += linked && r.dup_rev ? 1 : 0; chain += list && linked && !copy ? 1 : 0;
+			(copy ? copied : hashed) += in ? r.len - k + 1 : 0;
+			if (list) {
+				const uint32_t at = wave_append_slot(&list[0], in && !copy);
+				if (in && !copy) list[1 + at] = (uint32_t)ri;
+			}
+		}
+		wave_sum_add(&st[PSTAT_LINKS], links); wave_sum_add(&st[PSTAT_LINKS_REV], links_rev); wave_sum_add(&st[PSTAT_CHAIN], chain);
+		wave_sum_add(&st[PSTAT_HASHED], hashed); wave_sum_add(&st[PSTAT_COPIED], copied);
+	}
+};
+template <int NW>
+struct FPrepCheck {
+	Params p; const ContigRec* recs; uint32_t first; const uint8_t* pool; const uint64_t* kh; uint64_t* st;
+	ABG_HDN void operator()(uint64_t i, uint32_t lane, uint32_t nlanes) const
+	{
+		const ContigRec& rec = recs[first + i];
+		if (!dup_takes_copy(recs, rec, first)) return;
+		const uint8_t* seq = pool + rec.seq_off;
+		const uint64_t* have = kh + rec.seq_off;
+		const uint32_t cnk = rec.len - p.k + 1;
+		uint64_t bad = 0;
+		for (uint32_t j0 = lane * PREP_RUN; j0 < cnk; j0 += nlanes * PREP_RUN)
+			kmer_hash_run(p, [&](unsigned q) { return (unsigned)seq[q]; }, j0, j0 + PREP_RUN < cnk ? j0 + PREP_RUN : cnk,
+			    [&](uint32_t j, uint64_t h) { bad += have[j] != h ? 1 : 0; });
+		if (bad) atomic_add_u64(&st[PSTAT_MISMATCH], bad);
 	}
 };
 constexpr uint32_t PC_SCAN_RUN = 4;
@@ -2845,6 +3013,8 @@
 		if (memo_tab_.hmin) free_tab(memo_tab_);
 		if (plane_) be_.free(plane_);
 		if (wstats_) be_.free(wstats_);
+		if (pstat_) be_.free(pstat_);
+		if (plist_) be_.free(plist_);
 	}
 	void reset()
 	{
@@ -2867,6 +3037,7 @@
 		}
 		cend_count_ = 0;
 		if (wstats_) clear_wstats();
+		if (pstat_) be_.memset(pstat_, 0, PSTAT_N * 8);
 		ovf_seen_[0] = ovf_seen_[1] = 0;
 		if (gtab_.hmin) { free_tab(gtab_); gtab_ = WalkTab{ nullptr, nullptr, nullptr, 0 }; gtab_used_ = 0; }
 	}
@@ -3355,10 +3526,19 @@
 	               uint64_t bulk_calls = 0, bulk_steps = 0, lin_steps = 0, guide_slots = 0, chain_steps = 0, batch_cuts = 0, overflows = 0, memo_hits = 0, memo_adds = 0;
 	               uint64_t tiled_ops = 0, tiled_pending = 0, tile_overflows = 0, cls_covered_reads = 0, archive_bases = 0, cls_decided_reads = 0;
 	               uint64_t lead_stores[2] = { 0, 0 };
-	               uint64_t commit_rounds_incremental = 0, commit_dirty_records = 0, commit_first_chunk_decided = 0; };
+	               uint64_t commit_rounds_incremental = 0, commit_dirty_records = 0, commit_first_chunk_decided = 0;
+	               uint64_t dup_links = 0, dup_links_rev = 0, prep_hashed_kmers = 0, prep_copied_kmers = 0, prep_chain_rehashed = 0, prep_copy_mismatch = 0;
+	               uint64_t dup_scan_cut = 0;
+	};
 	Stats stats()
 	{
 		Stats s = stats_;
+		if (pstat_) {
+			uint64_t v[PSTAT_N];
+			be_.d2h(v, pstat_, sizeof v);
+			s.dup_links = v[PSTAT_LINKS]; s.dup_links_rev = v[PSTAT_LINKS_REV]; s.prep_hashed_kmers = v[PSTAT_HASHED];
+			s.prep_copied_kmers = v[PSTAT_COPIED]; s.prep_chain_rehashed = v[PSTAT_CHAIN]; s.prep_copy_mismatch = v[PSTAT_MISMATCH]; s.dup_scan_cut = v[PSTAT_CUT];
+		}
 		if (wstats_) {
 			uint64_t v[WSTAT_N];
 			be_.d2h(v, wstats_, sizeof v);
@@ -3498,6 +3678,8 @@
 	Guide guide_{ nullptr, 0, nullptr, 0, nullptr }; uint64_t* guide_tab_ = nullptr; uint32_t guide_log2_ = 0;
 	uint8_t* guide_seen_ = nullptr; uint64_t guide_seen_bytes_ = 0;
 	BulkScratch* bulk_pool_ = nullptr; uint64_t* wstats_ = nullptr; uint64_t guide_slots_ = 0;
+	uint32_t* plist_ = nullptr; uint32_t plist_cap_ = 0;
+	uint64_t* pstat_ = nullptr;
 	SuccMemo memo_{ nullptr, nullptr, nullptr, 0 }; WalkTab memo_tab_{ nullptr, nullptr, nullptr, 0 }; bool memo_valid_ = false; uint64_t memo_gen_ = 0;
 	bool walk_ready_ = false;
 	WalkTab wtab_{}, cend_{ nullptr, nullptr, nullptr, 0 };
@@ -4114,7 +4296,7 @@
 		walk_buf_cap_ = cfg_.buf_cap;
 		alloc_walk_scratch();
 		pool_cap_ = cfg_.pool_cap;
-		pool_ = (uint8_t*)be_.alloc(pool_cap_);
+		pool_ = (uint8_t*)be_.alloc(pool_cap_ + POOL_PAD);
 		kh_ = (uint64_t*)be_.alloc(pool_cap_ * 8);
 		pool_used_ = (uint64_t*)be_.alloc(8);
 		rec_cap_ = cfg_.rec_cap;
@@ -4168,7 +4350,7 @@
 		alloc_tab(wtab_, wtab_log2_);
 		be_.free(pool_); be_.free(kh_);
 		pool_cap_ *= 2;
-		pool_ = (uint8_t*)be_.alloc(pool_cap_);
+		pool_ = (uint8_t*)be_.alloc(pool_cap_ + POOL_PAD);
 		kh_ = (uint64_t*)be_.alloc(pool_cap_ * 8);
 		if (cfg_.verbose)
 			fprintf(stderr, "abyss_amd: walker resources grown: %u frames, %u bases, 2^%u table, %llu pool\n",
@@ -4458,7 +4640,7 @@
 		if (g_pool_ + tot_pool > pool_cap_) {
 			uint64_t cap = pool_cap_;
 			while (g_pool_ + tot_pool > cap) cap *= 2;
-			pool_ = (uint8_t*)regrow(pool_, pool_cap_, cap);
+			pool_ = (uint8_t*)regrow(pool_, pool_cap_, cap + POOL_PAD);
 			kh_ = (uint64_t*)regrow(kh_, pool_cap_ * 8, cap * 8);
 			pool_cap_ = cap;
 		}
@@ -4509,21 +4691,46 @@
 		be_.d2h(&nrec, rec_used_, 4);
 		nrec = std::min(nrec, rec_cap_);
 		if (nrec > prepped) {
-			FContigPrep<NW> f{ p_, cnt_, recs_, prepped, pool_, kh_, use_par_commit() ? 0u : 1u };
-			be_.launch_wave(nrec - prepped, f, "contig_prep");
-			if (use_par_commit()) link_duplicates(prepped, nrec);
+			const uint32_t nnew = nrec - prepped;
+			const bool par = use_par_commit();
+			const bool on_bases = par && cfg_.dup_bases && cfg_.link_duplicates && !dist() && !p_.mask;
+			if (on_bases) {
+				{ FDupFp f{ recs_, prepped, (const uint64_t*)pool_, (pool_cap_ + POOL_PAD) / 8 - 1, p_.k }; be_.launch_wave(nnew, f, "dup_link"); }
+				link_duplicates(prepped, nrec, true);
+				if (nnew + 1 > plist_cap_) {
+					if (plist_) be_.free(plist_);
+					plist_cap_ = std::max<uint32_t>(2 * (nnew + 1), 1024);
+					plist_ = (uint32_t*)be_.alloc(plist_cap_ * 4ull);
+				}
+				be_.memset(plist_, 0, 4);
+				{ FPrepList f{ recs_, p_.k, prepped, nrec, plist_, prep_stats() }; be_.launch_wave((nnew + 63) / 64, f, "contig_prep"); }
+				{ FContigPrep<NW> f{ p_, cnt_, recs_, prepped, pool_, kh_, 0u, plist_ }; be_.launch_wave(nnew, f, "contig_prep"); }
+				{ FDupCopy f{ recs_, kh_, p_.k, prepped }; be_.launch_wave(nnew, f, "contig_prep"); }
+				if (cfg_.prep_check) { FPrepCheck<NW> f{ p_, recs_, prepped, pool_, kh_, prep_stats() }; be_.launch_wave(nnew, f, "contig_prep"); }
+			} else {
+				FContigPrep<NW> f{ p_, cnt_, recs_, prepped, pool_, kh_, par ? 0u : 1u };
+				be_.launch_wave(nnew, f, "contig_prep");
+				if (par) link_duplicates(prepped, nrec, false);
+			}
+			if (par && !dist() && !on_bases) { FPrepList f{ recs_, p_.k, prepped, nrec, nullptr, prep_stats() }; be_.launch_wave((nnew + 63) / 64, f, "dup_link"); }
 			prepped = nrec;
 		}
 	}
-	void link_duplicates(uint32_t first_new, uint32_t nrec)
+	uint64_t* prep_stats()
+	{
+		if (!pstat_) { pstat_ = (uint64_t*)be_.alloc(PSTAT_N * 8); be_.memset(pstat_, 0, PSTAT_N * 8); }
+		return pstat_;
+	}
+	void link_duplicates(uint32_t first_new, uint32_t nrec, bool on_bases)
 	{
 		if (!cfg_.link_duplicates || dist() || nrec <= first_new || nrec < 2) return;
 		uint64_t* key = (uint64_t*)be_.alloc(nrec * 16ull); uint64_t* key2 = key + nrec;
 		uint32_t* val = (uint32_t*)be_.alloc(nrec * 8ull); uint32_t* val2 = val + nrec;
 		{ FDupKeys f{ recs_, p_.k, key, val }; be_.launch(nrec, f, "dup_link"); }
 		be_.sort_pairs_u64_u32(key, key2, val, val2, nrec);
-		{ FDupLink f{ recs_, key2, val2, nrec, first_new }; be_.launch(nrec, f, "dup_link"); }
-		{ FDupVerify f{ recs_, kh_, p_.k, first_new }; be_.launch_wave(nrec - first_new, f, "dup_link"); }
+		{ FDupLink f{ recs_, key2, val2, nrec, first_new, prep_stats() + PSTAT_CUT }; be_.launch(nrec, f, "dup_link"); }
+		if (on_bases) { FDupVerifyBases f{ recs_, (const uint64_t*)pool_, (pool_cap_ + POOL_PAD) / 8 - 1, first_new }; be_.launch_wave(nrec - first_new, f, "dup_link"); }
+		else { FDupVerify f{ recs_, kh_, p_.k, first_new }; be_.launch_wave(nrec - first_new, f, "dup_link"); }
 		be_.sync();
 		be_.free(key); be_.free(val);
 	}
@@ -4841,7 +5048,7 @@
 				if (pool_out) {
 					be_.free(pool_); be_.free(kh_);
 					pool_cap_ *= 2;
-					pool_ = (uint8_t*)be_.alloc(pool_cap_);
+					pool_ = (uint8_t*)be_.alloc(pool_cap_ + POOL_PAD);
 					kh_ = (uint64_t*)be_.alloc(pool_cap_ * 8);
 					if (cfg_.verbose) fprintf(stderr, "abyss_amd: contig pool grown to %llu bases\n", (unsigned long long)pool_cap_);
 				}
diff --git a/abyss_amd/csrc/abg_host.h b/abyss_amd/csrc/abg_host.h
--- a/abyss_amd/csrc/abg_host.h
+++ b/abyss_amd/csrc/abg_host.h
@@ -103,6 +103,8 @@
 		if (const char* e = getenv("ABG_COSETTLE_PASSES")) cfg.cosettle_passes = (uint32_t)std::max(1, atoi(e));
 		if (const char* e = getenv("ABG_COSETTLE_LOG2")) cfg.cosettle_log2 = (uint32_t)std::min(25, std::max(5, atoi(e)));
 		if (const char* e = getenv("ABG_LINK_DUPS")) cfg.link_duplicates = atoi(e) != 0;
+		if (const char* e = getenv("ABG_DUP_BASES")) cfg.dup_bases = atoi(e) != 0;
+		if (const char* e = getenv("ABG_PREP_CHECK")) cfg.prep_check = atoi(e) != 0;
 		if (const char* e = getenv("ABG_OVERLAP_PURITY")) cfg.overlap_purity = atoi(e) != 0;
 		if (const char* e = getenv("ABG_LEAD_IMPLICIT")) cfg.lead_implicit = atoi(e) != 0;
 		if (const char* e = getenv("ABG_APPLY_MASK")) cfg.apply_mask = atoi(e) != 0;
diff --git a/abyss_amd/csrc/abg_kernels.hip b/abyss_amd/csrc/abg_kernels.hip
--- a/abyss_amd/csrc/abg_kernels.hip
+++ b/abyss_amd/csrc/abg_kernels.hip
@@ -1130,6 +1130,9 @@
 		out->counter_bytes_held = ctx->s.eng->counter_bytes_held();
 		out->commit_rounds_incremental = s.commit_rounds_incremental; out->commit_dirty_records = s.commit_dirty_records;
 		out->commit_first_chunk_decided = s.commit_first_chunk_decided;
+		out->dup_links = s.dup_links; out->dup_links_rev = s.dup_links_rev; out->prep_hashed_kmers = s.prep_hashed_kmers;
+		out->prep_copied_kmers = s.prep_copied_kmers; out->prep_chain_rehashed = s.prep_chain_rehashed; out->prep_copy_mismatch = s.prep_copy_mismatch;
+		out->dup_scan_cut = s.dup_scan_cut;
 		return ABG_OK;
 	});
 }
diff --git a/abyss_amd/csrc/abg_walk.h b/abyss_amd/csrc/abg_walk.h
--- a/abyss_amd/csrc/abg_walk.h
+++ b/abyss_amd/csrc/abg_walk.h
@@ -111,6 +111,7 @@
 	uint32_t ins_prev;
 	uint32_t dup_of;
 	uint64_t fp;
+	uint8_t dup_rev;
 };
 constexpr uint32_t REC_END = 0xFFFFFFFFu;
 
@@ -923,7 +924,7 @@
 			rec.left_ext = lext; rec.right_ext = rext;
 			rec.left_code = (uint8_t)lcode; rec.right_code = (uint8_t)rcode;
 			rec.redundant = 0; rec.pre_redundant = 0; rec.coverage = 0; rec.contig_id = ~0ULL;
-			rec.ins_prev = 0; rec.dup_of = REC_END; rec.fp = 0;
+			rec.ins_prev = 0; rec.dup_of = REC_END; rec.fp = 0; rec.dup_rev = 0;
 			if (last == REC_END) first = ri; else e.recs[last].next = ri;
 			last = ri;
 			if (npopped) {
diff --git a/include/abyss_amd.h b/include/abyss_amd.h
--- a/include/abyss_amd.h
+++ b/include/abyss_amd.h
@@ -176,6 +176,13 @@
 	uint64_t commit_rounds_incremental;
 	uint64_t commit_dirty_records;
 	uint64_t commit_first_chunk_decided;
+	uint64_t dup_links;
+	uint64_t dup_links_rev;
+	uint64_t prep_hashed_kmers;
+	uint64_t prep_copied_kmers;
+	uint64_t prep_chain_rehashed;
+	uint64_t prep_copy_mismatch;
+	uint64_t dup_scan_cut;
 } abg_stats;
 int abg_get_stats(const abg_ctx* ctx, abg_stats* out);
 
```

After: 1680, median of 5. About the same (+0.2%).
